# endernewton/tf-faster-rcnn

Measured on AMD Instinct MI355X. Metric: images/sec (600×1000) ResNet-101 Faster R-CNN at 1/2/4/8 MI355X, higher is better.
Workload: dtype f32 (operands, accumulators, results; GEMMs with Cin, Cout % 128 == 0 form each f32 product from two-piece fp16 operands with an exact power-of-two scale per 128-k block on the fp16 matrix pipe -- 3 MFMAs / product, dropped terms <= 3 * 2^-22, measured error vs float64 below the f32-MFMA kernel's; o

## Files before the change

include/frcnn_hip.h:

```cpp
#ifndef FRCNN_HIP_H_
#define FRCNN_HIP_H_
#include <stddef.h>
#include <stdint.h>

#ifdef __cplusplus
extern "C" {
#endif

#define FRCNN_OK 0
#define FRCNN_E_ARG (-1)
#define FRCNN_E_WS (-2)
#define FRCNN_E_UNSUPPORTED (-3)
#define FRCNN_E_HIP(e) (-(1000 + (int)(e)))

#define FRCNN_NMS_RULE_CPU 0
#define FRCNN_NMS_RULE_GPU 1

#define FRCNN_ACT_NONE 0
#define FRCNN_ACT_RELU 1
#define FRCNN_ACT_RELU6 2

#define FRCNN_ABI_VERSION 6
int frcnn_abi_version(void);
const char* frcnn_build_info(void);
// ... 87 lines not shown
int frcnn_box_vote_host(const float* kept , int m, const float* cands , int n, double vote_thresh, float* out );
int frcnn_mirror_views(const float* in_d, int B, int OH, int OW, int c, float* out_d, void* stream);
int frcnn_merge_flip_views(const float* cls_prob_d, const float* bbox_pred_d, const float* rois_d, const int* num_rois_d, int B, int R,
                           int C, float im_w_scaled, float* out_prob_d, float* out_pred_d, float* out_rois_d, int* out_num_d,
                           void* stream);
int frcnn_merge_flip_views_host(const float* cls_prob, const float* bbox_pred, const float* rois, const int* num_rois, int B, int R, int C,
                                float im_w_scaled, float* out_prob, float* out_pred, float* out_rois, int* out_num);

int frcnn_im_detect_boxes(const float* rois_d, const float* bbox_pred_d, int R, int C, double im_scale,
                          int im_h, int im_w, float* boxes_d, void* stream);

int frcnn_bbox_transform_inv(const float* boxes_d, const float* deltas_d, int N, int k, float* out_d, void* stream);
int frcnn_clip_boxes(float* boxes_d, int N, int k, float im_h, float im_w, void* stream);
int frcnn_bbox_transform(const float* ex_rois_d, const float* gt_rois_d, int N, float* targets_d, void* stream);

int frcnn_bbox_overlaps(const double* boxes_d, int n, const double* query_d, int k, double* out_d, void* stream);

size_t frcnn_coco_match_workspace_bytes(int n_groups, long long n_det, long long n_gt, long long n_pairs);
int frcnn_coco_match(const double* det_xywh_d, const long long* det_off_d, const double* gt_xywh_d, const double* gt_area_d,
                     const unsigned char* gt_crowd_d, const long long* gt_off_d, int n_groups, const double* iou_thrs_d, int T,
                     const double* area_rng_d, int A, unsigned char* det_matched_d, unsigned char* det_ignored_d,
                     unsigned char* gt_ignored_d, double* iou_out_d, void* ws, size_t ws_bytes, void* stream);

size_t frcnn_proposal_recall_workspace_bytes(int n_images, long long max_boxes, long long n_gt_total);
int frcnn_proposal_recall(const float* boxes_d, int box_stride, long long n_rows, const long long* start_d, const int* count_d,
                          const float* scale_d, int n_images, long long max_boxes, int limit, const double* gt_d,
                          const long long* gt_off_d, long long n_gt_total, double* gt_iou_d, int* ran_out_d, void* ws, size_t ws_bytes,
                          void* stream);
int frcnn_proposal_recall_host(const float* boxes, int box_stride, long long n_rows, const long long* start, const int* count,
                               const float* scale, int n_images, long long max_boxes, int limit, const double* gt,
                               const long long* gt_off, long long n_gt_total, double* gt_iou, int* ran_out, void* ws, size_t ws_bytes);

int frcnn_conv2d_nhwc(const float* x_d, int N, int H, int W, int Cin, const float* w_d, const float* bias_d,
                      const float* residual_d, int RH, int RW, int res_stride, float* y_d, int OH, int OW,
                      int Cout, int KH, int KW, int stride, int pad_top, int pad_left, int act, int fold_w,
                      void* stream);
size_t frcnn_conv2d_workspace_bytes(int N, int OH, int OW, int Cout, int KH, int KW, int Cin, int fold_w);
int frcnn_conv2d_nhwc_ws(const float* x_d, int N, int H, int W, int Cin, const float* w_d, const float* bias_d,
                         const float* residual_d, int RH, int RW, int res_stride, float* y_d, int OH, int OW, int Cout, int KH,
                         int KW, int stride, int pad_top, int pad_left, int act, int fold_w, void* ws, size_t ws_bytes,
                         void* stream);

int frcnn_set_tuning(int key, int value);
unsigned int frcnn_crc32c(const void* data, size_t n, unsigned int crc);

long long frcnn_snappy_uncompress(const unsigned char* src, size_t n, unsigned char* dst, size_t cap);

int frcnn_prep_image_shape(int h, int w, int target_size, int max_size, double* im_scale, int* out_h, int* out_w);
int frcnn_prep_image(const void* src_d, int src_is_float, int h, int w, const double* pixel_means, double im_scale, float* out_d,
                     int OH, int OW, int out_c, void* stream);
int frcnn_prep_image_batched(const void* src_d, int src_is_float, int B, int h, int w, const double* pixel_means, double im_scale,
                             float* out_d, int OH, int OW, int out_c, void* stream);
int frcnn_prep_train_image(const void* src_d, int src_is_float, int h, int w, int flipped, const double* pixel_means, double im_scale,
                           float* out_d, int OH, int OW, int out_c, const unsigned short* boxes_d, const int* classes_d, int G,
                           float* gt_d, void* stream);

int frcnn_jpeg_info(const unsigned char* data, size_t n, int* out8);
size_t frcnn_jpeg_coef_bytes(int width, int height, int ncomp, int hs, int vs);
int frcnn_jpeg_entropy_decode(const unsigned char* data, size_t n, void* coef_h, size_t coef_bytes);
int frcnn_jpeg_pixels_host(const void* coef_h, int width, int height, int ncomp, int hs, int vs, unsigned char* bgr_h);
size_t frcnn_jpeg_workspace_bytes(int width, int height, int ncomp, int hs, int vs);
int frcnn_jpeg_pixels(const void* coef_d, int width, int height, int ncomp, int hs, int vs, unsigned char* bgr_d, void* ws,
                      size_t ws_bytes, void* stream);

int frcnn_jpeg_quant_tables(int quality, unsigned short* out128);
int frcnn_jpeg_coefs(const unsigned char* bgr_d, int width, int height, int hs, int vs, int quality, void* coef_d, void* ws,
                     size_t ws_bytes, void* stream);
int frcnn_jpeg_coefs_host(const unsigned char* bgr_h, int width, int height, int hs, int vs, int quality, void* coef_h);
size_t frcnn_jpeg_stream_bound(int width, int height, int hs, int vs);
long long frcnn_jpeg_entropy_encode(const void* coef_h, int width, int height, int hs, int vs, unsigned char* out, size_t cap);

int frcnn_draw_detections(unsigned char* bgr_d, int h, int w, const float* dets_d, const int* cnt_d, int max_dets, float conf,
                          int thickness, int scale, const unsigned char* colours_d, int num_colours, const unsigned char* labels_d,
                          int num_classes, int label_stride, const unsigned char* glyphs_d, void* stream);
int frcnn_draw_detections_host(unsigned char* bgr_h, int h, int w, const float* dets_h, int count, int max_dets, float conf,
                               int thickness, int scale, const unsigned char* colours_h, int num_colours, const unsigned char* labels_h,
                               int num_classes, int label_stride, const unsigned char* glyphs_h);

int frcnn_gemm_batched_nt(const float* x_d, const float* w_d, float* y_d, int G, int M, int N, int K, void* stream);
size_t frcnn_gemm_x3_pack_bytes(int G, int N, int K);
int frcnn_gemm_x3_pack(const float* w_d, int G, int N, int K, void* planes_d, void* stream);
int frcnn_gemm_x3(const float* x_d, const void* planes_d, const float* bias_d, const float* res_d, float* y_d, int G, int M, int N,
                  int K, int act, int cfg, int terms, void* stream);
size_t frcnn_h2_planes_bytes(long long rows, int K);
int frcnn_h2_pack_w(const float* w_d, int G, int N, int K, void* planes_d, float* w_inv_d, void* stream);
int frcnn_h2_split(const float* x_d, long long M, int K, void* planes_d, float* inv_d, void* stream);
int frcnn_gemm_h2(const void* x_planes_d, const float* x_inv_d, const void* w_planes_d, const float* w_inv_d, const float* bias_d,
                  const float* res_d, const void* res_planes_d, const float* res_inv_d, float* y_d, void* y_planes_d, float* y_inv_d,
                  int G, int M, int N, int K, int act, int cfg, void* stream);
size_t frcnn_gemm_h2_mean_workspace_bytes(int G, int M, int N);
int frcnn_gemm_h2_mean(const void* x_planes_d, const float* x_inv_d, const void* w_planes_d, const float* w_inv_d, const float* bias_d,
                       const float* res_d, const void* res_planes_d, const float* res_inv_d, int G, int M, int N, int K, int act, int rows,
                       float* mean_out_d, void* ws, size_t ws_bytes, int cfg, void* stream);
int frcnn_winograd_filter_transform(const float* w_hwio, int Cin, int Cout, const float* scale, int m, float* u_out);
int frcnn_winograd_filter_transform_device(const float* w_packed_d, int Cout, int Cin, int m, int transpose_flip, float* u_d,
                                           void* stream);
int frcnn_winograd_input_transform(const float* x_d, int N, int H, int W, int C, int m, float* v_d, void* stream);
int frcnn_winograd_output_transform(const float* m_d, int N, int H, int W, int C, int m, const float* bias_d, int act, float* y_d,
                                    void* stream);
int frcnn_winograd2_conv_x3(const float* x_d, int N, int H, int W, const void* u_planes_d, const float* bias_d, int act, float* y_d,
                            void* stream);
int frcnn_winograd7_filter_transform(const float* w_hwio, int Cin, int Cout, const float* scale, float* u_out);
int frcnn_winograd7_filter_transform_device(const float* w_packed_d, int Cout, int Cin, int transpose_flip, float* u_d, void* stream);
int frcnn_winograd7_input_transform(const float* x_d, int R, int C, float* v_d, void* stream);
int frcnn_winograd7_output_transform(const float* m_d, int R, int C, const float* bias_d, int act, float* y_d, void* stream);
int frcnn_winograd_input_transform_h2(const float* x_d, int N, int H, int W, int C, int m, void* v_planes_d, float* v_inv_d, void* stream);
int frcnn_winograd_output_transform_h2(const float* m_d, int N, int H, int W, int C, int m, const float* bias_d, int act, float* y_d,
                                       void* y_planes_d, float* y_inv_d, void* stream);
int frcnn_winograd7_input_transform_h2(const float* x_d, int R, int C, void* v_planes_d, float* v_inv_d, void* stream);
int frcnn_winograd7_output_transform_h2(const float* m_d, int R, int C, const float* bias_d, int act, float* y_d, void* y_planes_d,
                                        float* y_inv_d, void* stream);
int frcnn_pack_filter_hwio(const float* w_hwio, int KH, int KW, int Cin, int Cout, const float* scale, float* out);
int frcnn_maxpool_nhwc(const float* x_d, int N, int H, int W, int C, int k, int stride, int pad_top,
                       int pad_left, float* y_d, int OH, int OW, void* stream);
int frcnn_dwconv3x3_nhwc(const float* x_d, int N, int H, int W, int C, const float* w_d, const float* bias_d,
                         float* y_d, int OH, int OW, int stride, int pad_top, int pad_left, int act, void* stream);
int frcnn_dwconv3x3_nhwc_h2(const float* x_d, int N, int H, int W, int C, const float* w_d, const float* bias_d, float* y_d,
                            void* y_planes_d, float* y_inv_d, int OH, int OW, int stride, int pad_top, int pad_left, int act, void* stream);
int frcnn_spatial_mean(const float* x_d, int N, int HW, int C, float* y_d, void* stream);
int frcnn_softmax_rows(const float* x_d, int R, int C, int ld, float* y_d, void* stream);
int frcnn_rpn_softmax(const float* score_d, int HW, int A, int ld, float* prob_d, void* stream);
int frcnn_copy_cols(const float* src_d, int R, int ld_src, int col0, int cols, float* dst_d, int ld_dst, void* stream);

size_t frcnn_anchor_target_workspace_bytes(int H, int W, int A, int max_gt);
int frcnn_anchor_target_layer(const float* gt_boxes_d, int G, float im_h, float im_w, int H, int W, int A,
                              int feat_stride, const double* base_d, int rpn_batchsize, double fg_fraction,
                              double pos_overlap, double neg_overlap, long long seed, const double* opts, float* labels_d,
                              float* bbox_targets_d, float* inside_w_d, float* outside_w_d, void* ws,
                              size_t ws_bytes, void* stream);
int frcnn_anchor_target_layer_inject(const float* gt_boxes_d, int G, float im_h, float im_w, int H, int W, int A, int feat_stride,
                                     const double* base_d, int rpn_batchsize, double fg_fraction, double pos_overlap,
                                     double neg_overlap, const int* disable_d, int n_disable, const double* opts, float* labels_d,
                                     float* bbox_targets_d, float* inside_w_d, float* outside_w_d, void* ws, size_t ws_bytes,
                                     void* stream);
int frcnn_proposal_target_layer(const float* rpn_rois_d, const float* rpn_scores_d, int N, const float* gt_boxes_d,
                                int G, int num_classes, int batch_size, double fg_fraction, double fg_thresh,
                                double bg_thresh_hi, double bg_thresh_lo, const double* means4, const double* stds4,
                                long long seed, const double* opts, float* rois_d, float* roi_scores_d, float* labels_d,
                                float* bbox_targets_d, float* inside_w_d, float* outside_w_d, int* counts_d,
                                void* stream);
int frcnn_proposal_target_layer_dn(const float* rpn_rois_d, const float* rpn_scores_d, int max_rois, const int* num_rois_d,
                                   const float* gt_boxes_d, int G, int num_classes, int batch_size, double fg_fraction,
                                   double fg_thresh, double bg_thresh_hi, double bg_thresh_lo, const double* means4,
                                   const double* stds4, long long seed, const double* opts, float* rois_d, float* roi_scores_d,
                                   float* labels_d, float* bbox_targets_d, float* inside_w_d, float* outside_w_d, int* counts_d,
                                   void* stream);
int frcnn_proposal_target_layer_inject(const float* rpn_rois_d, const float* rpn_scores_d, int N, const float* gt_boxes_d, int G,
                                       int num_classes, int batch_size, const int* keep_inds_d, int n_fg, const double* means4,
                                       const double* stds4, const double* opts, float* rois_d, float* roi_scores_d, float* labels_d,
                                       float* bbox_targets_d, float* inside_w_d, float* outside_w_d, void* stream);
size_t frcnn_loss_workspace_bytes(long long elements);
int frcnn_softmax_ce_loss(const float* logits_d, const float* labels_d, int R, int C, int rpn_A, int rpn_H, int rpn_W,
                          float* loss_d, float* dlogits_d, void* ws, size_t ws_bytes, void* stream);
int frcnn_smooth_l1_loss(const float* pred_d, const float* targets_d, const float* inside_w_d, const float* outside_w_d,
                         long long n, float sigma, float mean_divisor, float* loss_d, float* dpred_d, void* ws,
                         size_t ws_bytes, void* stream);

int frcnn_transpose_pad(const float* in_d, int M, int C, float* out_d, int Mp, void* stream);
int frcnn_im2col_t(const float* x_d, int N, int H, int W, int Cin, int OH, int OW, int KH, int KW, int stride,
                   int pad_top, int pad_left, float* out_d, int Mp, void* stream);
int frcnn_flip_transpose_filter(const float* w_d, int Cout, int KH, int KW, int Cin, float* out_d, void* stream);
int frcnn_conv2d_dgrad_strided(const float* dy_d, int N, int OH, int OW, int Cout, const float* w_d, int KH, int KW,
                               int Cin, int stride, int pad_top, int pad_left, float* dx_d, int H, int W,
                               int accumulate, void* stream);
int frcnn_conv2d_wgrad_supported(int Cin, int Cout);
size_t frcnn_conv2d_wgrad_workspace_bytes(int N, int OH, int OW, int Cin, int Cout, int KH, int KW);
int frcnn_conv2d_wgrad(const float* dy_d, const float* x_d, int N, int H, int W, int Cin, int OH, int OW, int Cout, int KH, int KW,
                       int stride, int pad_top, int pad_left, float* dw_d, void* ws, size_t ws_bytes, void* stream);
void frcnn_conv2d_wgrad_set_plan(int tile, int min_workgroups);
size_t frcnn_conv2d_wgrad_h2_workspace_bytes(int N, int OH, int OW, int Cin, int Cout, int KH, int KW);
int frcnn_conv2d_wgrad_h2(const float* dy_d, const float* x_d, int N, int H, int W, int Cin, int OH, int OW, int Cout, int KH, int KW,
                          int stride, int pad_top, int pad_left, float* dw_d, void* ws, size_t ws_bytes, void* stream);
// ... 63 lines not shown
```

tf-faster-rcnn_amd/csrc/gemm_h2.hip:

```cpp
#include "h2_common.h"
#include <mutex>
#include <type_traits>

typedef float f32x16 __attribute__((ext_vector_type(16)));
typedef _Float16 h8 __attribute__((ext_vector_type(8)));

#define LDS_AS __attribute__((address_space(3)))

struct GemmH2Params {
  const unsigned short* x; const float* x_inv; const unsigned short* w; const float* w_inv;
  const float* bias; const float* res; const unsigned short* resp; const float* resp_inv; float* y; unsigned short* yp; float* y_inv;
  int M, N, K, batch, act, nsteps, mtiles, ntiles;
  long long Mtot;
  int wshare;
  const float* mask;
  float* mean_part; int mean_rows;
};

__device__ __forceinline__ void h2_glds16(unsigned voff, const void* sbase, unsigned lds_base) {
  unsigned keep;
  asm volatile(
      "s_mov_b32 %0, m0\n\t"
      "s_mov_b32 m0, %3\n\t"
      "s_nop 0\n\t"
      "global_load_lds_dwordx4 %1, %2\n\t"
      "s_mov_b32 m0, %0"
      : "=&s"(keep)
      : "v"(voff), "s"(sbase), "s"(lds_base)
      : "memory");
}

__device__ __forceinline__ void h2_glds4(unsigned voff, const void* sbase, unsigned lds_base) {
  unsigned keep;
  asm volatile(
      "s_mov_b32 %0, m0\n\t"
      "s_mov_b32 m0, %3\n\t"
      "s_nop 0\n\t"
      "global_load_lds_dword %1, %2\n\t"
      "s_mov_b32 m0, %0"
      : "=&s"(keep)
      : "v"(voff), "s"(sbase), "s"(lds_base)
      : "memory");
}

__device__ __forceinline__ void h2_glds16c(unsigned voff, const void* sbase, unsigned lds_base) {
  asm volatile(
      "s_mov_b32 m0, %2\n\t"
      "s_nop 0\n\t"
      "global_load_lds_dwordx4 %0, %1"
      :
      : "v"(voff), "s"(sbase), "s"(lds_base)
      : "memory");
}
__device__ __forceinline__ void h2_glds4c(unsigned voff, const void* sbase, unsigned lds_base) {
  asm volatile(
      "s_mov_b32 m0, %2\n\t"
      "s_nop 0\n\t"
      "global_load_lds_dword %0, %1"
      :
      : "v"(voff), "s"(sbase), "s"(lds_base)
      : "memory");
}

template <int N>
__device__ __forceinline__ void h2_wait_vmcnt() {
  asm volatile("s_waitcnt vmcnt(%0)" ::"n"(N) : "memory");
}

enum H2Tune : int {
  H2_SCALES_ONCE = 2,
  H2_PINGPONG = 32,
  H2_MASKED = 128,
  H2_LIGHT_BOUNDARY = 256,
  H2_STORE16 = 512,
  H2_DEFERRED = 1024,
#ifdef FRCNN_ABLATION
  H2_NO_MFMA = 2048,
  H2_NO_FRAG = 4096,
  H2_NO_LOAD = 8192,
#endif
};

template <int BM, int BN, int WM, int WN, int NS, int TUNE>
struct H2Lds {
  static constexpr int NW = (BM / WM) * (BN / WN);
  static constexpr bool PP = (TUNE & H2_PINGPONG) != 0;
  static constexpr int XP = BM * 64, WP = BN * 64;
  static constexpr int S_OFF = 2 * XP + 2 * WP;
  static constexpr int STAGE = S_OFF + (PP ? 0 : 1024);
  static constexpr int RED_OFF = NS * STAGE;
  static constexpr int S2_OFF = RED_OFF + (BN / WN) * BM * 4;
  static constexpr int CB_OFF = S2_OFF + (PP ? NW * 512 : (TUNE & H2_SCALES_ONCE) ? 2048 : 0);
  static constexpr int TOTAL = CB_OFF + ((TUNE & H2_LIGHT_BOUNDARY) ? 2 * 2 * BN * 4 : 0);
  static constexpr int RI_OFF = S_OFF + 512;
};

template <int BM, int BN, int WM, int WN, int NS, int WPE = 2, int TUNE = 0>
__global__ __launch_bounds__((BM / WM) * (BN / WN) * 64) __attribute__((amdgpu_waves_per_eu(WPE))) void k_gemm_h2(const GemmH2Params p) {
  constexpr int NW = (BM / WM) * (BN / WN);
  constexpr int TM = WM / 32, TN = WN / 32;
  constexpr int LA = 2 * BM / 16 / NW;
  constexpr int LB = 2 * BN / 16 / NW;
  constexpr int G = LA + LB;
  constexpr int SL = BM / 64;
  constexpr bool ONCE = (TUNE & H2_SCALES_ONCE) != 0;
  constexpr bool PP = (TUNE & H2_PINGPONG) != 0;
  constexpr bool MASKED = (TUNE & H2_MASKED) != 0;
  constexpr bool LTB = (TUNE & H2_LIGHT_BOUNDARY) != 0;
  constexpr bool W21 = (TUNE & H2_STORE16) != 0;
  constexpr bool DE = (TUNE & H2_DEFERRED) != 0;
  using L = H2Lds<BM, BN, WM, WN, NS, TUNE>;
  constexpr int XP = L::XP, WP = L::WP, S_OFF = L::S_OFF, STAGE = L::STAGE, RED_OFF = L::RED_OFF, S2_OFF = L::S2_OFF, CB_OFF = L::CB_OFF, RI_OFF = L::RI_OFF;
  static_assert(!LTB || (!PP && NS == 2 && NW >= 4 && BN % 64 == 0 && BM <= 128), "light boundary: the two-slot one-barrier-per-slab schedule");
  static_assert(!DE || (LTB && W21 && BN == H2_KB), "deferred epilogue: built on the light boundary's LDS constants and counted waits");
  static_assert(!PP || (NW == 8 && NS == 3 && ONCE && BM == 256 && WM == 64 && BN == 128 && WN == 64),
                "ping-pong geometry: 8 waves as 4 (M) x 2 (N), waves 0-3 = the upper half of the rows");
  static_assert((2 * BM / 16) % NW == 0 && (2 * BN / 16) % NW == 0, "tile/wave mismatch");
  static_assert(BM <= 256 && NS >= 2 && NS <= 4, "stage layout");
  static_assert((NS - 2) * (G + SL) <= 63, "vmcnt range");
  extern __shared__ __attribute__((aligned(16))) char smem[];

  const int tid = threadIdx.x, lane = tid & 63;
  const int wave = __builtin_amdgcn_readfirstlane(tid >> 6);
  const int per = p.mtiles * p.ntiles, T = per * p.batch;
  const int xcd = blockIdx.x & 7, wx = blockIdx.x >> 3, W8 = gridDim.x >> 3;
  const int tq = T / 8, tr = T % 8, tn = tq + (xcd < tr ? 1 : 0);
  const int t_end = (xcd < tr ? xcd * (tq + 1) : tr * (tq + 1) + (xcd - tr) * tq) + tn;
  const int tile0 = t_end - tn + wx;
  if (tile0 >= t_end) return;
  const int my_tiles = (t_end - tile0 + W8 - 1) / W8;
  int left = __builtin_amdgcn_readfirstlane(my_tiles * p.nsteps);

  const int wmi = wave / (BN / WN), wni = wave % (BN / WN);
  const int wm0 = wmi * WM, wn0 = wni * WN;
  const int frow = lane & 31, khalf = lane >> 5;

  const size_t xplane = (size_t)p.Mtot * p.K * 2, wplane = (size_t)p.N * p.K * 2;
  unsigned a_off[LA], b_off[LB], s_off[SL];
  const char* i_xb = nullptr; const char* i_wb = nullptr; const char* i_sb = nullptr;
  int i_tile = tile0, i_step = 0, i_par = 0, c_par = 0;
  int i_g = 0, i_bm0 = 0, i_bn0 = 0, i_cpar = 0, c_cpar = 0;
  int pend = 0;
#pragma unroll
  for (int t = 0; t < LB; ++t) {
    const int u = wave * LB + t, plane = u / (BN / 16), row = (u % (BN / 16)) * 16 + (lane >> 2), pos = lane & 3;
    b_off[t] = (unsigned)((size_t)plane * wplane + (size_t)row * p.K * 2 + ((pos ^ ((row >> 2) & 3)) * 16));
  }
  auto tile_coords = [&](int tl, int& g, int& mt, int& nt) {
    g = tl / per;
    const int rem = tl - g * per;
    mt = rem / p.ntiles;
    nt = rem - mt * p.ntiles;
  };
  auto set_tile = [&](int tl) {
    int g, mt, nt;
    tile_coords(tl, g, mt, nt);
    const int bm0 = mt * BM, bn0 = nt * BN;
    const size_t row0 = (size_t)g * p.M + bm0;
    i_g = g; i_bm0 = bm0; i_bn0 = bn0;
    i_xb = (const char*)p.x + row0 * p.K * 2;
    i_wb = (const char*)p.w + ((size_t)(p.wshare ? 0 : g) * 2 * p.N + bn0) * p.K * 2;
    i_sb = (const char*)(p.x_inv + row0);
#pragma unroll
    for (int t = 0; t < LA; ++t) {
      const int u = wave * LA + t, plane = u / (BM / 16), row = (u % (BM / 16)) * 16 + (lane >> 2), pos = lane & 3;
      const int rr = min(row, p.M - 1 - bm0);
      a_off[t] = (unsigned)((size_t)plane * xplane + (size_t)rr * p.K * 2 + ((pos ^ ((row >> 2) & 3)) * 16));
    }
    const long long last = p.Mtot - 1 - (long long)row0;
#pragma unroll
    for (int j = 0; j < SL; ++j) s_off[j] = (unsigned)(min((long long)((PP ? wm0 : j * 64) + lane), last) * 4);
  };
  const unsigned lds0 = (unsigned)(size_t)(LDS_AS char*)smem;
  auto uniform_ptr = [](const char* q) {
    const unsigned long long v = (unsigned long long)q;
    const unsigned lo = __builtin_amdgcn_readfirstlane((unsigned)v), hi = __builtin_amdgcn_readfirstlane((unsigned)(v >> 32));
    return (const char*)(((unsigned long long)hi << 32) | lo);
  };
  auto issue_one = [&](int buf, int t) {
    const unsigned sb = lds0 + (unsigned)(buf * STAGE);
    if constexpr (PP) {
      if (t < LA) h2_glds16c(a_off[t], uniform_ptr(i_xb), __builtin_amdgcn_readfirstlane(sb + (wave * LA + t) * 1024));
      else if (t < G) h2_glds16c(b_off[t - LA], uniform_ptr(i_wb), __builtin_amdgcn_readfirstlane(sb + 2 * XP + (wave * LB + (t - LA)) * 1024));
      else if (t == G && (i_step & 3) == 0) {
        h2_glds4c(s_off[0], uniform_ptr(i_sb), __builtin_amdgcn_readfirstlane(lds0 + S2_OFF + (wave * 2 + i_par) * 256));
        i_par ^= 1;
      }
      return;
    }
    if (t < LA) h2_glds16(a_off[t], uniform_ptr(i_xb), __builtin_amdgcn_readfirstlane(sb + (wave * LA + t) * 1024));
    else if (t < G) h2_glds16(b_off[t - LA], uniform_ptr(i_wb), __builtin_amdgcn_readfirstlane(sb + 2 * XP + (wave * LB + (t - LA)) * 1024));
    else if (wave == 0) {
      const int j = t - G;
      if (!ONCE) h2_glds4(s_off[j], uniform_ptr(i_sb), __builtin_amdgcn_readfirstlane(sb + S_OFF + j * 256));
      else if ((i_step & 3) == 0) {
        h2_glds4(s_off[j], uniform_ptr(i_sb), __builtin_amdgcn_readfirstlane(lds0 + S2_OFF + i_par * 1024 + j * 256));
        if (j == SL - 1) i_par ^= 1;
      }
    }
  };
  static_assert(!ONCE || NS == 2 || PP, "scales-once needs the uncounted wait of the two-stage ring");
  auto issue_advance = [&]() {
    --left;
    if (++i_step == p.nsteps) {
      i_step = 0; i_tile += W8;
      if (left > 0) set_tile(i_tile);
    } else {
      i_xb += 64; i_wb += 64;
      if ((i_step & 3) == 0) i_sb += (size_t)p.Mtot * 4;
    }
  };

  auto issue_cb = [&]() {
    const unsigned cb = lds0 + CB_OFF + i_cpar * (2 * BN * 4);
    if (wave == 1) {
#pragma unroll
      for (int j = 0; j < BN / 64; ++j)
        h2_glds4((unsigned)(lane * 4), uniform_ptr((const char*)(p.w_inv + (size_t)(p.wshare ? 0 : i_g) * p.N + i_bn0 + j * 64)),
                 __builtin_amdgcn_readfirstlane(cb + j * 256));
    }
    if (wave == 2 && p.bias) {
#pragma unroll
      for (int j = 0; j < BN / 64; ++j)
        h2_glds4((unsigned)(lane * 4), uniform_ptr((const char*)(p.bias + i_bn0 + j * 64)), __builtin_amdgcn_readfirstlane(cb + BN * 4 + j * 256));
    }
    if (wave == 3 && p.resp) {
      const char* rb = (const char*)(p.resp_inv + (size_t)(i_bn0 / H2_KB) * p.Mtot + (size_t)i_g * p.M + i_bm0);
#pragma unroll
      for (int j = 0; j < SL; ++j)
        h2_glds4((unsigned)(min(j * 64 + lane, p.M - 1 - i_bm0) * 4), uniform_ptr(rb), __builtin_amdgcn_readfirstlane(lds0 + i_cpar * STAGE + RI_OFF + j * 256));
    }
    i_cpar ^= 1;
  };
  auto wait_pending = [&](int n) {
    if constexpr (DE) {
      if (n >= 32) {
        if (n >= 48) { if (n >= 56) h2_wait_vmcnt<56>(); else h2_wait_vmcnt<48>(); }
        else { if (n >= 40) h2_wait_vmcnt<40>(); else h2_wait_vmcnt<32>(); }
      } else {
        if (n >= 16) { if (n >= 24) h2_wait_vmcnt<24>(); else h2_wait_vmcnt<16>(); }
        else { if (n >= 8) h2_wait_vmcnt<8>(); else h2_wait_vmcnt<0>(); }
      }
      return;
    }
    if (n >= 63) h2_wait_vmcnt<63>();
    else if (n >= 48) h2_wait_vmcnt<48>();
    else if (n >= 32) h2_wait_vmcnt<32>();
    else if (n >= 16) h2_wait_vmcnt<16>();
    else h2_wait_vmcnt<0>();
  };

  f32x16 tot[TM][TN], tmp[TM][TN];
  const int sw = (frow >> 2) & 3;
  const int x_row = (wm0 + frow) * 64, w_row = 2 * XP + (wn0 + frow) * 64;

#ifdef FRCNN_ABLATION
  constexpr bool NO_MFMA = (TUNE & H2_NO_MFMA) != 0, NO_FRAG = (TUNE & H2_NO_FRAG) != 0, NO_LOAD = (TUNE & H2_NO_LOAD) != 0;
#else
  constexpr bool NO_MFMA = false, NO_FRAG = false, NO_LOAD = false;
#endif
  h8 kxh[NO_FRAG ? TM : 1], kxl[NO_FRAG ? TM : 1], kwh[NO_FRAG ? TN : 1], kwl[NO_FRAG ? TN : 1];
  (void)kxh; (void)kxl; (void)kwh; (void)kwl;
  auto slab_mfma = [&](int cur, auto first_c) {
    constexpr bool FIRST = decltype(first_c)::value;
    const char* sb = smem + cur * STAGE;
#pragma unroll
    for (int t = 0; t < 2; ++t) {
      h8 xh[TM], xl[TM], wh[TN], wl[TN];
      if constexpr (NO_FRAG) {
        if (FIRST && t == 0) {
#pragma unroll
          for (int j = 0; j < TN; ++j) {
            const char* q = sb + w_row + j * 32 * 64 + ((khalf ^ sw) * 16);
            kwh[j] = __builtin_bit_cast(h8, *(const uint4*)(q));
            kwl[j] = __builtin_bit_cast(h8, *(const uint4*)(q + WP));
          }
#pragma unroll
          for (int i = 0; i < TM; ++i) {
            const char* q = sb + x_row + i * 32 * 64 + ((khalf ^ sw) * 16);
            kxh[i] = __builtin_bit_cast(h8, *(const uint4*)(q));
            kxl[i] = __builtin_bit_cast(h8, *(const uint4*)(q + XP));
          }
        }
#pragma unroll
        for (int j = 0; j < TN; ++j) { wh[j] = kwh[j]; wl[j] = kwl[j]; asm volatile("" : "+v"(wh[j]), "+v"(wl[j])); }
#pragma unroll
        for (int i = 0; i < TM; ++i) { xh[i] = kxh[i]; xl[i] = kxl[i]; asm volatile("" : "+v"(xh[i]), "+v"(xl[i])); }
      } else {
#pragma unroll
      for (int j = 0; j < TN; ++j) {
        const char* q = sb + w_row + j * 32 * 64 + (((2 * t + khalf) ^ sw) * 16);
        wh[j] = __builtin_bit_cast(h8, *(const uint4*)(q));
        wl[j] = __builtin_bit_cast(h8, *(const uint4*)(q + WP));
      }
#pragma unroll
      for (int i = 0; i < TM; ++i) {
        const char* q = sb + x_row + i * 32 * 64 + (((2 * t + khalf) ^ sw) * 16);
// ... 372 lines not shown
        if (live) ep_rowmax_merge(mx);
      }
      if (live) {
#pragma unroll
        for (int i = 0; i < TM; ++i) ep_store_planes(T, i, mx[i]);
      }
      if (BN / WN > 1) {
        asm volatile("s_waitcnt lgkmcnt(0)" ::: "memory");
        __builtin_amdgcn_s_barrier();
      }
    }
    c_cpar ^= 1;
  };

  constexpr int HALF = (TM + 1) / 2;
  bool have_prev = false;
  TileRef P{0, 0, 0, 0};
  float dmx[TM];
  (void)dmx;
  auto de_piece = [&](auto pos_c) {
    constexpr int POS = decltype(pos_c)::value;
    if constexpr (POS == 0) {
      if (have_prev) {
        ep_scale_act(P);
        ep_mask(P);
        if (p.yp) ep_rowmax_write(dmx);
      }
    } else if constexpr (POS == 1 || POS == 2) {
      constexpr int I0 = POS == 1 ? 0 : HALF, I1 = POS == 1 ? HALF : TM;
      if (have_prev) {
        if (POS == 1 && p.yp && BN / WN > 1) ep_rowmax_merge(dmx);
#pragma unroll
        for (int i = I0; i < I1; ++i) {
          ep_store_f32(P, i);
          if (p.yp) ep_store_planes(P, i, dmx[i]);
        }
      }
#pragma unroll
      for (int i = I0; i < I1; ++i) load_res_raw(i);
    }
  };

  auto slab = [&](auto pos_c, bool fold, bool first_block) {
    constexpr int POS = decltype(pos_c)::value;
    const std::integral_constant<bool, POS == 0> first_c{};
    if constexpr (DE) asm volatile("s_waitcnt lgkmcnt(0)" ::: "memory");
    if constexpr (LTB) {
      wait_pending(pend);
    } else if (left >= 1) {
      if (wave == 0) h2_wait_vmcnt<(NS - 2) * (G + SL)>(); else h2_wait_vmcnt<(NS - 2) * G>();
    } else {
      h2_wait_vmcnt<0>();
    }
    __builtin_amdgcn_s_barrier();
    const bool more = left > 0;
    if (more) {
#pragma unroll
      for (int t = 0; t < (NO_LOAD ? 0 : G + SL); ++t) issue_one(nxt, t);
      if constexpr (LTB) {
        if (i_step == 0) issue_cb();
        pend = 0;
      }
    }
    if constexpr (DE) {
      __builtin_amdgcn_sched_barrier(0);
      if (first_block) de_piece(pos_c);
      __builtin_amdgcn_sched_barrier(0);
    }
    float ainv[TM];
    if (fold) {
      const int soff = ONCE ? S2_OFF + c_par * 1024 : cur * STAGE + S_OFF;
#pragma unroll
      for (int i = 0; i < TM; ++i) ainv[i] = *(const float*)(smem + soff + (wm0 + i * 32 + frow) * 4);
      c_par ^= 1;
    }
    slab_mfma(cur, first_c);
    if (more) {
      issue_advance();
      nxt = nxt + 1 == NS ? 0 : nxt + 1;
    }
    if (fold) {
      if (LTB && first_block) {
        const float* cbp = (const float*)(smem + CB_OFF + c_cpar * (2 * BN * 4));
        if (!p.res && p.resp) {
          typedef unsigned u32x2 __attribute__((ext_vector_type(2)));
#pragma unroll
          for (int i = 0; i < TM; ++i) {
            const float rri = *(const float*)(smem + c_cpar * STAGE + RI_OFF + (wm0 + i * 32 + frow) * 4);
#pragma unroll
            for (int j = 0; j < TN; ++j)
#pragma unroll
              for (int pq = 0; pq < 2; ++pq) {
                unsigned w[8];
#pragma unroll
                for (int e = 0; e < 8; ++e) w[e] = __float_as_uint(tot[i][j][8 * pq + e]);
                const auto h0 = __builtin_amdgcn_permlane32_swap(w[0], w[2], false, false), h1 = __builtin_amdgcn_permlane32_swap(w[1], w[3], false, false);
                const auto l0 = __builtin_amdgcn_permlane32_swap(w[4], w[6], false, false), l1 = __builtin_amdgcn_permlane32_swap(w[5], w[7], false, false);
                const h4 ha = __builtin_bit_cast(h4, u32x2{h0[0], h1[0]}), hb = __builtin_bit_cast(h4, u32x2{h0[1], h1[1]});
                const h4 la = __builtin_bit_cast(h4, u32x2{l0[0], l1[0]}), lb = __builtin_bit_cast(h4, u32x2{l0[1], l1[1]});
#pragma unroll
                for (int e = 0; e < 4; ++e) {
                  tot[i][j][8 * pq + e] = ((float)ha[e] + (float)la[e]) * rri;
                  tot[i][j][8 * pq + 4 + e] = ((float)hb[e] + (float)lb[e]) * rri;
                }
              }
          }
        }
#pragma unroll
        for (int j = 0; j < TN; ++j)
#pragma unroll
          for (int q = 0; q < 4; ++q) {
            const float4 wi = *(const float4*)(cbp + wn0 + j * 32 + 4 * khalf + 8 * q);
            const float4 bv = p.bias ? *(const float4*)(cbp + BN + wn0 + j * 32 + 4 * khalf + 8 * q) : make_float4(0.f, 0.f, 0.f, 0.f);
            const float s0 = __uint_as_float(0x7f000000u - __float_as_uint(wi.x)), s1 = __uint_as_float(0x7f000000u - __float_as_uint(wi.y));
            const float s2 = __uint_as_float(0x7f000000u - __float_as_uint(wi.z)), s3 = __uint_as_float(0x7f000000u - __float_as_uint(wi.w));
#pragma unroll
            for (int i = 0; i < TM; ++i) {
              tot[i][j][4 * q + 0] = __builtin_fmaf(tmp[i][j][4 * q + 0], ainv[i], (tot[i][j][4 * q + 0] + bv.x) * s0);
              tot[i][j][4 * q + 1] = __builtin_fmaf(tmp[i][j][4 * q + 1], ainv[i], (tot[i][j][4 * q + 1] + bv.y) * s1);
              tot[i][j][4 * q + 2] = __builtin_fmaf(tmp[i][j][4 * q + 2], ainv[i], (tot[i][j][4 * q + 2] + bv.z) * s2);
              tot[i][j][4 * q + 3] = __builtin_fmaf(tmp[i][j][4 * q + 3], ainv[i], (tot[i][j][4 * q + 3] + bv.w) * s3);
            }
          }
      } else {
#pragma unroll
        for (int i = 0; i < TM; ++i)
#pragma unroll
          for (int j = 0; j < TN; ++j)
#pragma unroll
            for (int r = 0; r < 16; ++r) tot[i][j][r] = __builtin_fmaf(tmp[i][j][r], ainv[i], tot[i][j][r]);
      }
    }
    cur = cur + 1 == NS ? 0 : cur + 1;
  };

  set_tile(i_tile);
  set_ctile(c_tile);
  if constexpr (PP) {
    const int grp = wave >> 2;
    h8 fxh[2][TM], fxl[2][TM], fwh[2][TN], fwl[2][TN];
    auto seg_barrier = [&]() {
      __builtin_amdgcn_sched_barrier(0);
      __builtin_amdgcn_s_barrier();
      __builtin_amdgcn_sched_barrier(0);
    };
    auto fold = [&]() {
      float ainv[TM];
#pragma unroll
      for (int i = 0; i < TM; ++i) ainv[i] = *(const float*)(smem + S2_OFF + (wave * 2 + c_par) * 256 + (i * 32 + frow) * 4);
      c_par ^= 1;
#pragma unroll
      for (int i = 0; i < TM; ++i)
#pragma unroll
        for (int j = 0; j < TN; ++j)
#pragma unroll
          for (int r = 0; r < 16; ++r) tot[i][j][r] = __builtin_fmaf(tmp[i][j][r], ainv[i], tot[i][j][r]);
    };
    auto pp_mem = [&](auto pos_c, bool fold_prev, bool live) -> bool {
      constexpr int POS = decltype(pos_c)::value;
      const char* sb = smem + cur * STAGE;
      if (live) {
#pragma unroll
        for (int t = 0; t < 2; ++t) {
#pragma unroll
          for (int j = 0; j < TN; ++j) {
            const char* q = sb + w_row + j * 32 * 64 + (((2 * t + khalf) ^ sw) * 16);
            fwh[t][j] = __builtin_bit_cast(h8, *(const uint4*)(q));
            fwl[t][j] = __builtin_bit_cast(h8, *(const uint4*)(q + WP));
          }
#pragma unroll
          for (int i = 0; i < TM; ++i) {
            const char* q = sb + x_row + i * 32 * 64 + (((2 * t + khalf) ^ sw) * 16);
            fxh[t][i] = __builtin_bit_cast(h8, *(const uint4*)(q));
            fxl[t][i] = __builtin_bit_cast(h8, *(const uint4*)(q + XP));
          }
        }
      } else {
#pragma unroll
        for (int t = 0; t < 2; ++t) {
#pragma unroll
          for (int j = 0; j < TN; ++j) asm volatile("" : "=v"(fwh[t][j]), "=v"(fwl[t][j]));
#pragma unroll
          for (int i = 0; i < TM; ++i) asm volatile("" : "=v"(fxh[t][i]), "=v"(fxl[t][i]));
        }
      }
      const bool more = left > 0;
      if (more) {
#pragma unroll
        for (int t = 0; t <= G; ++t) issue_one(nxt, t);
        issue_advance();
        nxt = nxt + 1 == NS ? 0 : nxt + 1;
      }
      if (fold_prev) fold();
      if (grp == 1) {
        if (more) h2_wait_vmcnt<(POS == 2 ? G + 1 : G)>(); else h2_wait_vmcnt<0>();
      }
// ... 9 lines not shown
        for (int t = 0; t < 2; ++t) {
#pragma unroll
          for (int i = 0; i < TM; ++i)
#pragma unroll
            for (int j = 0; j < TN; ++j) {
              if (POS == 0 && t == 0) {
                f32x16 z;
#pragma unroll
                for (int r = 0; r < 16; ++r) z[r] = 0.f;
                tmp[i][j] = __builtin_amdgcn_mfma_f32_32x32x16_f16(fwh[t][j], fxh[t][i], z, 0, 0, 0);
              } else {
                tmp[i][j] = __builtin_amdgcn_mfma_f32_32x32x16_f16(fwh[t][j], fxh[t][i], tmp[i][j], 0, 0, 0);
              }
            }
#pragma unroll
          for (int i = 0; i < TM; ++i)
#pragma unroll
            for (int j = 0; j < TN; ++j) tmp[i][j] = __builtin_amdgcn_mfma_f32_32x32x16_f16(fwl[t][j], fxh[t][i], tmp[i][j], 0, 0, 0);
#pragma unroll
          for (int i = 0; i < TM; ++i)
#pragma unroll
            for (int j = 0; j < TN; ++j) tmp[i][j] = __builtin_amdgcn_mfma_f32_32x32x16_f16(fwh[t][j], fxl[t][i], tmp[i][j], 0, 0, 0);
        }
      }
      __builtin_amdgcn_s_setprio(0);
      if (grp == 0) {
        if (issued) h2_wait_vmcnt<(POS == 2 ? G + 1 : G)>(); else h2_wait_vmcnt<0>();
      }
      cur = cur + 1 == NS ? 0 : cur + 1;
      seg_barrier();
    };
    bool two = false;
#pragma unroll
    for (int s2 = 0; s2 < 2; ++s2) {
      if (left > 0) {
#pragma unroll
        for (int t = 0; t <= G; ++t) issue_one(nxt, t);
        issue_advance();
        nxt = nxt + 1 == NS ? 0 : nxt + 1;
        two = s2 == 1;
      }
    }
    if (two) h2_wait_vmcnt<G>(); else h2_wait_vmcnt<0>();
    seg_barrier();
    if (grp == 1) seg_barrier();
    const int nkb = p.nsteps >> 2;
    for (int tl = 0; tl < my_tiles; ++tl) {
      const bool live = __builtin_amdgcn_readfirstlane(c_bm0 + wm0 < p.M ? 1 : 0) != 0;
      if (live) init_tot();
      else {
#pragma unroll
        for (int i = 0; i < TM; ++i)
#pragma unroll
          for (int j = 0; j < TN; ++j) asm volatile("" : "=v"(tot[i][j]));
      }
      for (int kb = 0; kb < nkb; ++kb) {
        bool is;
        is = pp_mem(std::integral_constant<int, 0>{}, live && kb > 0, live); pp_mfma(std::integral_constant<int, 0>{}, is, live);
        is = pp_mem(std::integral_constant<int, 1>{}, false, live);          pp_mfma(std::integral_constant<int, 1>{}, is, live);
        is = pp_mem(std::integral_constant<int, 2>{}, false, live);          pp_mfma(std::integral_constant<int, 2>{}, is, live);
        is = pp_mem(std::integral_constant<int, 3>{}, false, live);          pp_mfma(std::integral_constant<int, 3>{}, is, live);
      }
      if (live) fold(); else c_par ^= nkb & 1;
      epilogue(live);
      c_tile += W8;
      if (tl + 1 < my_tiles) set_ctile(c_tile);
    }
    if (grp == 0) seg_barrier();
    h2_wait_vmcnt<0>();
    return;
  }
#pragma unroll
  for (int s = 0; s < NS - 1; ++s) {
    if (left > 0) {
#pragma unroll
      for (int t = 0; t < G + SL; ++t) issue_one(nxt, t);
      if constexpr (LTB) {
        if (i_step == 0) issue_cb();
        pend = 0;
      }
      issue_advance();
      nxt = nxt + 1 == NS ? 0 : nxt + 1;
    }
  }
  const int nkb = p.nsteps >> 2;
  for (int tl = 0; tl < my_tiles; ++tl) {
    init_tot();
    for (int kb = 0; kb < nkb; ++kb) {
      slab(std::integral_constant<int, 0>{}, false, kb == 0);
      slab(std::integral_constant<int, 1>{}, false, kb == 0);
      slab(std::integral_constant<int, 2>{}, false, kb == 0);
      slab(std::integral_constant<int, 3>{}, true, kb == 0);
    }
    if constexpr (DE) {
      if (tl + 1 < my_tiles) {
        P = TileRef{c_bm0, c_bn0, c_g, c_cpar};
        have_prev = true;
        c_cpar ^= 1;
        c_tile += W8;
        set_ctile(c_tile);
        continue;
      }
    }
    epilogue(true);
    c_tile += W8;
    if (tl + 1 < my_tiles) set_ctile(c_tile);
  }
  h2_wait_vmcnt<0>();
}

__global__ __launch_bounds__(256) void k_h2_split(const float* __restrict__ x, long long M, int K, unsigned short* __restrict__ planes,
                                                  float* __restrict__ inv_out) {
  const int nkb = K / H2_KB;
  const long long pairs = M * nkb;
  const int sub = threadIdx.x >> 5, l = threadIdx.x & 31;
  for (long long pr = (long long)blockIdx.x * 8 + sub; pr < pairs; pr += (long long)gridDim.x * 8) {
    const long long m = pr / nkb;
    const int kb = (int)(pr - m * nkb);
    const size_t e = (size_t)m * K + (size_t)kb * H2_KB + 4 * l;
    const float4 v = *(const float4*)(x + e);
    float mx = fmaxf(fmaxf(fabsf(v.x), fabsf(v.y)), fmaxf(fabsf(v.z), fabsf(v.w)));
#pragma unroll
    for (int o = 16; o >= 1; o >>= 1) mx = fmaxf(mx, __shfl_xor(mx, o, 64));
    float scale, inv;
    h2_block_scale(mx, scale, inv);
    h4 hh, ll;
    h2_split4(v, scale, hh, ll);
    *(h4*)(planes + e) = hh;
    *(h4*)(planes + (size_t)M * K + e) = ll;
    if (l == 0) inv_out[(size_t)kb * M + m] = inv;
  }
}

__global__ __launch_bounds__(256) void k_h2_pack_w(const float* __restrict__ w, int rows, int N, int K, unsigned short* __restrict__ planes,
                                                   float* __restrict__ inv_out) {
  const int row = blockIdx.x * 4 + (threadIdx.x >> 6), l = threadIdx.x & 63;
  if (row >= rows) return;
  const float* src = w + (size_t)row * K;
  float mx = 0.f;
  for (int k = 4 * l; k < K; k += 256) {
    const float4 v = *(const float4*)(src + k);
    mx = fmaxf(mx, fmaxf(fmaxf(fabsf(v.x), fabsf(v.y)), fmaxf(fabsf(v.z), fabsf(v.w))));
  }
#pragma unroll
  for (int o = 32; o >= 1; o >>= 1) mx = fmaxf(mx, __shfl_xor(mx, o, 64));
  float scale, inv;
  h2_block_scale(fmaxf(mx, 0x1p-40f), scale, inv);
  const int g = row / N, n = row - g * N;
  unsigned short* ph = planes + ((size_t)g * 2 * N + n) * K;
  unsigned short* pl = ph + (size_t)N * K;
  for (int k = 4 * l; k < K; k += 256) {
    const float4 v = *(const float4*)(src + k);
    h4 hh, ll;
    _Float16 a, b;
    h2_split1(v.x, scale, a, b); hh[0] = a; ll[0] = b;
    h2_split1(v.y, scale, a, b); hh[1] = a; ll[1] = b;
    h2_split1(v.z, scale, a, b); hh[2] = a; ll[2] = b;
    h2_split1(v.w, scale, a, b); hh[3] = a; ll[3] = b;
    *(h4*)(ph + k) = hh;
    *(h4*)(pl + k) = ll;
  }
  if (l == 0) inv_out[row] = inv;
}

extern "C" size_t frcnn_h2_planes_bytes(long long rows, int K) {
  if (rows <= 0 || K <= 0) return 0;
// ... 106 lines not shown
    return FRCNN_E_ARG;
  const long long Mtot = (long long)G * M;
  if (K % H2_KB || N % 128 || 4ll * Mtot * K >= (1ll << 32) || 4ll * N * K >= (1ll << 32) || (long long)M * N >= (1ll << 29)) return FRCNN_E_UNSUPPORTED;
  GemmH2Params p = h2_params(x_planes_d, x_inv_d, w_planes_d, w_inv_d, bias_d, res_d, nullptr, nullptr, y_d, y_planes_d, y_inv_d, G, M, N, K, act);
  p.mask = mask_d;
  return run_h2(p, cfg, (hipStream_t)stream);
}

static int run_h2(GemmH2Params& p, int cfg, hipStream_t st) {
  const int G = p.batch, M = p.M, N = p.N, K = p.K;
  if (cfg < 0) {
    const bool classes = cfg == -1;
    if (cfg == -9) cfg = -1;
    const long long mt256 = (M + 255) / 256, t256 = mt256 * (N / 128) * G;
#ifndef FRCNN_H2_PP_MIN_K
#define FRCNN_H2_PP_MIN_K 1024
#endif
    const int pp_min_k = ((cfg == -4 || cfg == -5 || cfg == -6) && !p.mean_part) ? 512 : FRCNN_H2_PP_MIN_K;
    int pp_cfg = (cfg == -3 || cfg == -4 || (cfg == -6 && K < FRCNN_H2_PP_MIN_K)) ? 34 : 21;
    const bool waste256_ok = mt256 * 256 * 100 <= (long long)M * 104;
    bool pp = K >= pp_min_k && waste256_ok && t256 >= 256;
    bool to31 = false;
    if (classes && !p.mean_part && !p.mask) {
      const long long m64 = (M + 63) / 64 * 64;
      const bool waste64_ok = m64 * 100 <= (long long)M * 104;
      const bool products = (FRCNN_H2_PP_CLASSES & 1) && G > 1 && p.y && !p.yp && !p.res && !p.resp && K >= 512 && waste64_ok && t256 >= 256;
      const bool conv3_f32res = (FRCNN_H2_PP_CLASSES & 2) && p.res && p.yp && K == 512 && waste64_ok && t256 >= 256;
      if (conv3_f32res && !pp) pp_cfg = 34;
      pp = pp || products || conv3_f32res;
      to31 = (FRCNN_H2_PP_CLASSES & 4) && p.resp && p.yp && !p.y && K == 512;
    }
    const bool tiny = (long long)((M + 127) / 128) * (N / 128) * G < 150;
    const bool de = cfg != -2 && cfg != -7 && !p.mean_part && !p.mask && ((p.resp && p.yp && !p.y) || cfg == -8) && !to31;
    cfg = pp ? pp_cfg : tiny ? (cfg == -2 ? 12 : (de && cfg == -8) ? 41 : 33) : (cfg == -2 ? 9 : de ? 40 : 31);
  }
  if (p.mean_part && (cfg == 40 || cfg == 41)) cfg = cfg == 40 ? 31 : 33;
  return p.mask ? h2_dispatch<H2_MASKED>(p, cfg, st) : h2_dispatch<0>(p, cfg, st);
}

__global__ __launch_bounds__(256) void k_h2_mean_finish(const float* __restrict__ part, int G, int M, int N4, int rows, float4* __restrict__ out) {
  const long long t = (long long)blockIdx.x * blockDim.x + threadIdx.x;
  const int per = M / rows;
  if (t >= (long long)G * per * N4) return;
  const int n4 = (int)(t % N4);
  const long long gr = t / N4;
  const int g = (int)(gr / per), r = (int)(gr % per);
  const int nblk = (M + 31) >> 5;
  const int row0 = r * rows, row1 = row0 + rows - 1;
  float4 s = make_float4(0.f, 0.f, 0.f, 0.f);
  for (int b = row0 >> 5; b <= (row1 >> 5); ++b) {
    const int which = ((b << 5) / rows == r) ? 0 : 1;
    const float4 v = *(const float4*)(part + (((size_t)g * nblk + b) * 2 + which) * (size_t)N4 * 4 + (size_t)n4 * 4);
    s.x += v.x; s.y += v.y; s.z += v.z; s.w += v.w;
  }
  const float inv = 1.0f / (float)rows;
  out[t] = make_float4(s.x * inv, s.y * inv, s.z * inv, s.w * inv);
}

extern "C" size_t frcnn_gemm_h2_mean_workspace_bytes(int G, int M, int N) {
  if (G <= 0 || M <= 0 || N <= 0) return 256;
  return (size_t)G * (size_t)((M + 31) / 32) * 2 * (size_t)N * sizeof(float);
}

extern "C" int frcnn_gemm_h2_mean(const void* x_planes_d, const float* x_inv_d, const void* w_planes_d, const float* w_inv_d, const float* bias_d,
                                  const float* res_d, const void* res_planes_d, const float* res_inv_d, int G, int M, int N, int K, int act, int rows,
                                  float* mean_out_d, void* ws, size_t ws_bytes, int cfg, void* stream) {
  if (!x_planes_d || !x_inv_d || !w_planes_d || !w_inv_d || !mean_out_d || !ws || G <= 0 || M <= 0 || N <= 0 || K <= 0 || act < 0 || act > 2 ||
      rows <= 0 || (res_d && res_planes_d) || (res_planes_d && !res_inv_d))
    return FRCNN_E_ARG;
  const long long Mtot = (long long)G * M;
  if (K % H2_KB || N % 128 || M % rows || rows < 32 || 4ll * Mtot * K >= (1ll << 32) || 4ll * N * K >= (1ll << 32) || (long long)M * N >= (1ll << 29))
    return FRCNN_E_UNSUPPORTED;
  if (frcnn_gemm_h2_mean_workspace_bytes(G, M, N) > ws_bytes) return FRCNN_E_WS;
  GemmH2Params p = h2_params(x_planes_d, x_inv_d, w_planes_d, w_inv_d, bias_d, res_d, res_planes_d, res_inv_d, nullptr, nullptr, nullptr, G, M, N, K, act);
  p.mean_part = (float*)ws; p.mean_rows = rows; p.wshare = 1;
  hipStream_t st = (hipStream_t)stream;
  const int rc = run_h2(p, cfg, st);
  if (rc) return rc;
  const long long tot = (long long)G * (M / rows) * (N / 4);
  hipLaunchKernelGGL(k_h2_mean_finish, dim3((unsigned)((tot + 255) / 256)), dim3(256), 0, st, (const float*)ws, G, M, N / 4, rows, (float4*)mean_out_d);
  LAUNCH_CHECK();
  return FRCNN_OK;
}
```

tf-faster-rcnn_amd/csrc/gemm_x3.hip:

```cpp
#include "common.h"
#include "x3_mma.h"
#include <mutex>

struct GemmX3Params {
  const float* x; const unsigned short* wp; const float* bias; const float* res; float* y;
  int M, N, K, nsteps, mtiles, ntiles, batch, act;
  long long gx, gwp, gy;
};

template <int BM, int BN, int WM, int WN, int TERMS = 6>
__global__ __launch_bounds__((BM / WM) * (BN / WN) * 64) __attribute__((amdgpu_waves_per_eu(2))) void k_gemm_x3(const GemmX3Params p) {
  constexpr int NW = (BM / WM) * (BN / WN);
  constexpr int TM = WM / 32, TN = WN / 32;
  constexpr int LA = BM / 8 / NW;
  constexpr int LB = 3 * BN / 16 / NW;
  constexpr int G = LA + LB;
  constexpr int A_BYTES = BM * 128, P_BYTES = BN * 64, STAGE = A_BYTES + 3 * P_BYTES;
  static_assert((BM / 8) % NW == 0 && (3 * BN / 16) % NW == 0, "tile/wave mismatch");
  extern __shared__ __attribute__((aligned(16))) char smem[];

  const int tid = threadIdx.x, lane = tid & 63;
  const int wave = __builtin_amdgcn_readfirstlane(tid >> 6);
  const int per = p.mtiles * p.ntiles, T = per * p.batch;
  const int xcd = blockIdx.x & 7, wx = blockIdx.x >> 3, W8 = gridDim.x >> 3;
  const int tq = T / 8, tr = T % 8, tn = tq + (xcd < tr ? 1 : 0);
  const int t_end = (xcd < tr ? xcd * (tq + 1) : tr * (tq + 1) + (xcd - tr) * tq) + tn;
  int tile = __builtin_amdgcn_readfirstlane(t_end - tn + wx);
  if (tile >= t_end) return;

  const int wm0 = (wave / (BN / WN)) * WM, wn0 = (wave % (BN / WN)) * WN;
  int a_lane[LA], b_lane[LB];
#pragma unroll
  for (int t = 0; t < LB; ++t) {
    const int u = wave * LB + t;
    const int plane = u / (BN / 16), row = (u % (BN / 16)) * 16 + (lane >> 2), pos = lane & 3;
    b_lane[t] = ((plane * p.N + row) * p.K) * 2 + ((pos ^ ((row >> 2) & 3)) * 16);
  }
  const float* ia = p.x; const char* ib = (const char*)p.wp;
  int i_bm0 = 0, i_bn0 = 0, i_g = 0;
  auto set_tile = [&](int tl) {
    const int g = tl / per, rem = tl - g * per;
    const int mt = rem / p.ntiles, nt = rem - mt * p.ntiles;
    i_bm0 = mt * BM; i_bn0 = nt * BN; i_g = g;
    ia = p.x + (size_t)g * p.gx + (size_t)i_bm0 * p.K;
    ib = (const char*)(p.wp + (size_t)g * p.gwp + (size_t)i_bn0 * p.K);
#pragma unroll
    for (int t = 0; t < LA; ++t) {
      const int row = (wave * LA + t) * 8 + (lane >> 3);
      a_lane[t] = (min(row, p.M - 1 - i_bm0) * p.K + ((lane & 7) ^ ((row >> 1) & 7)) * 4) * 4;
    }
  };
  const unsigned lds0 = (unsigned)(size_t)(LDS_AS char*)smem;
  auto issue_one = [&](int buf, int t) {
    const unsigned sb = lds0 + (unsigned)(buf * STAGE);
    if (t < LA) glds16((const char*)ia + a_lane[t], __builtin_amdgcn_readfirstlane(sb + (wave * LA + t) * 1024));
    else glds16(ib + b_lane[t - LA], __builtin_amdgcn_readfirstlane(sb + A_BYTES + (wave * LB + (t - LA)) * 1024));
  };
  auto advance_k = [&]() { ia += 32; ib += 64; };
  auto issue_slab = [&](int buf) {
#pragma unroll
    for (int t = 0; t < G; ++t) issue_one(buf, t);
    advance_k();
  };

  f32x16 acc[TM][TN], acs[TM][TN];
  auto zero_acc = [&]() {
#pragma unroll
    for (int i = 0; i < TM; ++i)
#pragma unroll
      for (int j = 0; j < TN; ++j)
#pragma unroll
        for (int r = 0; r < 16; ++r) { acc[i][j][r] = 0.f; acs[i][j][r] = 0.f; }
  };
  zero_acc();
  const int frow = lane & 31, khalf = lane >> 5;
  const int a_sw = (frow >> 1) & 7, b_sw = (frow >> 2) & 3;
  const int a_row = (wm0 + frow) * 128, b_row = A_BYTES + (wn0 + frow) * 64;

  int c_bm0, c_bn0, c_g;
  const int lane_off = (4 * khalf * p.N + frow) * 4;
  auto sub_base = [&](int i, int j) { return (long long)(c_bm0 + wm0 + i * 32) * p.N + (long long)(c_bn0 + wn0 + j * 32); };
  auto row_soff = [&](int r) { return ((r & 3) + 8 * (r >> 2)) * p.N * 4; };
  auto rsrc_of = [&](const float* tensor, long long sbase) {
    const long long left = ((long long)p.M * p.N - sbase) * 4;
    return __builtin_amdgcn_make_buffer_rsrc((void*)(tensor + sbase), 0, (int)max(0ll, min(left, 0x7fffffffll)), 0x00020000);
  };

  auto slab_body = [&](int cur) {
    const int nbuf = cur ^ 1;
    const char* sb = smem + cur * STAGE;
#pragma unroll
    for (int t = 0; t < 2; ++t) {
      bf16x8 ah[TM], am[TM], al[TM], bh[TN], bm[TN], bl[TN];
#pragma unroll
      for (int j = 0; j < TN; ++j) {
        const char* q = sb + b_row + j * 32 * 64 + (((2 * t + khalf) ^ b_sw) * 16);
        bh[j] = __builtin_bit_cast(bf16x8, *(const uint4*)(q));
        bm[j] = __builtin_bit_cast(bf16x8, *(const uint4*)(q + P_BYTES));
        bl[j] = __builtin_bit_cast(bf16x8, *(const uint4*)(q + 2 * P_BYTES));
      }
#pragma unroll
      for (int i = 0; i < TM; ++i) {
        const char* q = sb + a_row + i * 32 * 128;
        const float4 f0 = *(const float4*)(q + (((4 * t + 2 * khalf) ^ a_sw) * 16));
        const float4 f1 = *(const float4*)(q + (((4 * t + 2 * khalf + 1) ^ a_sw) * 16));
        x3_split8(f0, f1, ah[i], am[i], al[i]);
      }
#pragma unroll
      for (int u = (t * G) / 2; u < ((t + 1) * G) / 2; ++u) issue_one(nbuf, u);
#pragma unroll
      for (int i = 0; i < TM; ++i)
#pragma unroll
        for (int j = 0; j < TN; ++j)
          x3_mma16<TERMS>(ah[i], am[i], al[i], bh[j], bm[j], bl[j], acc[i][j], acs[i][j]);
    }
    advance_k();
  };

  const float act_lo = p.act == FRCNN_ACT_NONE ? -__builtin_inff() : 0.f;
  const float act_hi = p.act == FRCNN_ACT_RELU6 ? 6.f : __builtin_inff();
  auto finish = [&](auto res_c) {
    constexpr bool RES = decltype(res_c)::value;
    float* const py = p.y + (size_t)c_g * p.gy;
    int lo = lane_off;
    asm volatile("" : "+v"(lo));
#pragma unroll
    for (int i = 0; i < TM; ++i)
#pragma unroll
      for (int j = 0; j < TN; ++j) {
        const float bv = p.bias ? p.bias[c_bn0 + wn0 + j * 32 + frow] : 0.f;
        const long long sbase = sub_base(i, j);
        float v[16];
        if (RES) {
          const auto rr = rsrc_of(p.res + (size_t)c_g * p.gy, sbase);
#pragma unroll
          for (int r = 0; r < 16; ++r) v[r] = __builtin_bit_cast(float, __builtin_amdgcn_raw_buffer_load_b32(rr, lo + row_soff(r), 0, 0));
        }
#pragma unroll
        for (int r = 0; r < 16; ++r) {
          float t = (acc[i][j][r] + acs[i][j][r]) + bv;
          if (RES) t += v[r];
          v[r] = act_clamp(t, act_lo, act_hi);
        }
        const auto ry = rsrc_of(py, sbase);
#pragma unroll
        for (int r = 0; r < 16; ++r) __builtin_amdgcn_raw_buffer_store_b32(__builtin_bit_cast(unsigned, v[r]), ry, lo + row_soff(r), 0, 0);
      }
  };

  set_tile(tile);
  c_bm0 = i_bm0; c_bn0 = i_bn0; c_g = i_g;
  issue_slab(0);
  int cur = 0, step = 0;
  for (;;) {
    wait_vmcnt<0>();
    __builtin_amdgcn_s_barrier();
    const bool last = step + 1 == p.nsteps;
    int next = tile;
    if (last) {
      next = __builtin_amdgcn_readfirstlane(tile + W8);
      set_tile(next < t_end ? next : tile);
    }
    slab_body(cur);
    cur ^= 1;
    if (!last) { ++step; continue; }
    if (p.res) finish(std::true_type{}); else finish(std::false_type{});
    if (next >= t_end) break;
    zero_acc();
    step = 0; tile = next; c_bm0 = i_bm0; c_bn0 = i_bn0; c_g = i_g;
  }
  wait_vmcnt<0>();
}

__global__ void k_x3_pack(const float* __restrict__ w, long long nk, int G, unsigned short* __restrict__ out) {
  const long long i = (long long)blockIdx.x * blockDim.x + threadIdx.x;
  if (i >= nk * G) return;
  const long long g = i / nk, e = i - g * nk;
  const float x = w[i];
  const __bf16 h = (__bf16)x;
  const float r = x - (float)h;
  const __bf16 m = (__bf16)r;
  const __bf16 l = (__bf16)(r - (float)m);
  unsigned short* o = out + (size_t)g * 3 * nk + e;
  o[0] = __builtin_bit_cast(unsigned short, h); o[nk] = __builtin_bit_cast(unsigned short, m); o[2 * nk] = __builtin_bit_cast(unsigned short, l);
}

extern "C" size_t frcnn_gemm_x3_pack_bytes(int G, int N, int K) {
  if (G <= 0 || N <= 0 || K <= 0) return 0;
  return (size_t)G * 3 * (size_t)N * (size_t)K * sizeof(unsigned short);
}

extern "C" int frcnn_gemm_x3_pack(const float* w_d, int G, int N, int K, void* planes_d, void* stream) {
  if (!w_d || !planes_d || G <= 0 || N <= 0 || K <= 0) return FRCNN_E_ARG;
  const long long nk = (long long)N * K, tot = nk * G;
  hipLaunchKernelGGL(k_x3_pack, dim3((unsigned)((tot + 255) / 256)), dim3(256), 0, (hipStream_t)stream, w_d, nk, G, (unsigned short*)planes_d);
  LAUNCH_CHECK();
  return FRCNN_OK;
}

template <int BM, int BN, int WM, int WN, int TERMS = 6>
static int launch_x3(const GemmX3Params& q, hipStream_t st) {
  constexpr int NT = (BM / WM) * (BN / WN) * 64;
  constexpr size_t lds = 2 * (size_t)(BM * 128 + 3 * BN * 64);
  auto kern = k_gemm_x3<BM, BN, WM, WN, TERMS>;
  static KernelOnce once;
  int slots = 0;
  HIP_TRY(kernel_once(once, (const void*)kern, NT, lds, &slots));
  if (slots < 8 || q.N % BN) return FRCNN_E_UNSUPPORTED;
  GemmX3Params p = q;
  p.mtiles = cdiv(p.M, BM); p.ntiles = p.N / BN; p.nsteps = p.K / 32;
  const long long T = (long long)p.mtiles * p.ntiles * p.batch;
  if (T >= (1ll << 30)) return FRCNN_E_UNSUPPORTED;
  const int grid = (int)min((long long)(slots / 8) * 8, ((T + 7) / 8) * 8);
  hipLaunchKernelGGL(kern, dim3(grid), dim3(NT), lds, st, p);
  LAUNCH_CHECK();
  return FRCNN_OK;
}

extern "C" int frcnn_gemm_x3(const float* x_d, const void* planes_d, const float* bias_d, const float* res_d, float* y_d, int G, int M,
                             int N, int K, int act, int cfg, int terms, void* stream) {
  if (!x_d || !planes_d || !y_d || G <= 0 || M <= 0 || N <= 0 || K <= 0 || act < 0 || act > 2 || (terms != 6 && terms != 9)) return FRCNN_E_ARG;
  if (K % 32 || N % 64 || (long long)M * N >= (1ll << 31) || (long long)N * K >= (1ll << 28) || K >= (1 << 22))
    return FRCNN_E_UNSUPPORTED;
  GemmX3Params p;
  p.x = x_d; p.wp = (const unsigned short*)planes_d; p.bias = bias_d; p.res = res_d; p.y = y_d;
  p.M = M; p.N = N; p.K = K; p.batch = G; p.act = act;
  p.gx = (long long)M * K; p.gwp = 3ll * N * K; p.gy = (long long)M * N;
  p.nsteps = p.mtiles = p.ntiles = 0;
  hipStream_t st = (hipStream_t)stream;
  if (cfg >= 0 && cfg < 10 && (N % 128) && cfg != 6) cfg = -1;
  if (cfg < 0)
    cfg = (N % 128) ? 6 : ((long long)cdiv(M, 128) * (N / 128) * G >= 256) ? 0 : 1;
  if (terms == 9) {
    switch (cfg) {
      case 0: return launch_x3<128, 128, 64, 64, 9>(p, st);
      case 1: return launch_x3<128, 128, 32, 64, 9>(p, st);
      case 6: return launch_x3<128, 64, 64, 32, 9>(p, st);
      default: return FRCNN_E_ARG;
    }
  }
  switch (cfg) {
    case 0: return launch_x3<128, 128, 64, 64>(p, st);
    case 1: return launch_x3<128, 128, 32, 64>(p, st);
    case 2: return launch_x3<64, 128, 32, 64>(p, st);
    case 3: return launch_x3<128, 128, 32, 128>(p, st);
    case 4: return launch_x3<256, 128, 64, 64>(p, st);
    case 5: return launch_x3<128, 256, 64, 64>(p, st);
    case 6: return launch_x3<128, 64, 64, 32>(p, st);
    default: return FRCNN_E_ARG;
  }
}
```

tf-faster-rcnn_amd/frcnn_hip/__init__.py:

```python
import ctypes
import os
from ctypes import c_double, c_float, c_int, c_longlong, c_size_t, c_ulonglong, c_void_p

_PKG = os.path.dirname(os.path.abspath(__file__))
LIB_PATH = os.path.join(_PKG, "libfrcnn_hip.so")
_lib = None

ABI_VERSION = 6
ACT_NONE, ACT_RELU, ACT_RELU6 = 0, 1, 2
NMS_RULE_CPU, NMS_RULE_GPU = 0, 1

_P = c_void_p
SIGNATURES = {
    "frcnn_abi_version": (c_int, []),
    "frcnn_build_info": (ctypes.c_char_p, []),
    "_nms": (None, [_P, _P, _P, c_int, c_int, c_float, c_int]),
    "frcnn_nms_workspace_bytes": (c_size_t, [c_int]),
    "frcnn_nms": (c_int, [_P, c_int, c_double, c_int, _P, _P, _P, c_size_t, _P]),
    "frcnn_nms_sorted": (c_int, [_P, c_int, c_int, c_double, c_int, _P, _P, _P, c_size_t, _P]),
    "frcnn_nms_rule": (c_int, [_P, c_int, c_double, c_int, c_int, _P, _P, _P, c_size_t, _P]),
    "frcnn_nms_sorted_rule": (c_int, [_P, c_int, c_int, c_double, c_int, c_int, _P, _P, _P, c_size_t, _P]),
    "frcnn_generate_anchors": (c_int, [c_int, _P, c_int, _P, c_int, _P]),
    "frcnn_generate_anchors_pre": (c_int, [c_int, c_int, c_int, _P, c_int, _P, _P]),
    "frcnn_proposal_workspace_bytes": (c_size_t, [c_int, c_int, c_int, c_int]),
# ... 46 lines not shown
    "frcnn_conv2d_nhwc": (c_int, [_P, c_int, c_int, c_int, c_int, _P, _P, _P, c_int, c_int, c_int, _P, c_int, c_int,
                                  c_int, c_int, c_int, c_int, c_int, c_int, c_int, c_int, _P]),
    "frcnn_conv2d_workspace_bytes": (c_size_t, [c_int, c_int, c_int, c_int, c_int, c_int, c_int, c_int]),
    "frcnn_conv2d_nhwc_ws": (c_int, [_P, c_int, c_int, c_int, c_int, _P, _P, _P, c_int, c_int, c_int, _P, c_int, c_int,
                                     c_int, c_int, c_int, c_int, c_int, c_int, c_int, c_int, _P, c_size_t, _P]),
    "frcnn_conv2d_nhwc_masked_ws": (c_int, [_P, c_int, c_int, c_int, c_int, _P, _P, _P, c_int, c_int, c_int, _P, c_int, c_int,
                                            c_int, c_int, c_int, c_int, c_int, c_int, c_int, _P, _P, c_size_t, _P]),
    "frcnn_gemm_h2_masked": (c_int, [_P, _P, _P, _P, _P, _P, _P, _P, _P, _P, c_int, c_int, c_int, c_int, c_int, c_int, _P]),
    "frcnn_winograd_output_transform_masked": (c_int, [_P, c_int, c_int, c_int, c_int, c_int, _P, _P, _P, _P, _P]),
    "frcnn_winograd7_output_transform_masked": (c_int, [_P, c_int, c_int, _P, _P, _P, _P, _P]),
    "frcnn_crc32c": (ctypes.c_uint32, [_P, c_size_t, ctypes.c_uint32]),
    "frcnn_snappy_uncompress": (c_longlong, [_P, c_size_t, _P, c_size_t]),
    "frcnn_prep_image_shape": (c_int, [c_int, c_int, c_int, c_int, _P, _P, _P]),
    "frcnn_prep_image": (c_int, [_P, c_int, c_int, c_int, _P, c_double, _P, c_int, c_int, c_int, _P]),
    "frcnn_prep_image_batched": (c_int, [_P, c_int, c_int, c_int, c_int, _P, c_double, _P, c_int, c_int, c_int, _P]),
    "frcnn_prep_train_image": (c_int, [_P, c_int, c_int, c_int, c_int, _P, c_double, _P, c_int, c_int, c_int, _P, _P, c_int, _P, _P]),
    "frcnn_jpeg_info": (c_int, [_P, c_size_t, _P]),
    "frcnn_jpeg_coef_bytes": (c_size_t, [c_int, c_int, c_int, c_int, c_int]),
    "frcnn_jpeg_entropy_decode": (c_int, [_P, c_size_t, _P, c_size_t]),
    "frcnn_jpeg_pixels_host": (c_int, [_P, c_int, c_int, c_int, c_int, c_int, _P]),
    "frcnn_jpeg_workspace_bytes": (c_size_t, [c_int, c_int, c_int, c_int, c_int]),
    "frcnn_jpeg_pixels": (c_int, [_P, c_int, c_int, c_int, c_int, c_int, _P, _P, c_size_t, _P]),
    "frcnn_jpeg_quant_tables": (c_int, [c_int, _P]),
    "frcnn_jpeg_coefs": (c_int, [_P, c_int, c_int, c_int, c_int, c_int, _P, _P, c_size_t, _P]),
    "frcnn_jpeg_coefs_host": (c_int, [_P, c_int, c_int, c_int, c_int, c_int, _P]),
    "frcnn_jpeg_stream_bound": (c_size_t, [c_int, c_int, c_int, c_int]),
    "frcnn_jpeg_entropy_encode": (c_longlong, [_P, c_int, c_int, c_int, c_int, _P, c_size_t]),
    "frcnn_draw_detections": (c_int, [_P, c_int, c_int, _P, _P, c_int, c_float, c_int, c_int, _P, c_int, _P, c_int, c_int, _P, _P]),
    "frcnn_draw_detections_host": (c_int, [_P, c_int, c_int, _P, c_int, c_int, c_float, c_int, c_int, _P, c_int, _P, c_int, c_int, _P]),
    "frcnn_gemm_batched_nt": (c_int,[_P, _P, _P, c_int, c_int, c_int, c_int, _P]),
    "frcnn_winograd_filter_transform": (c_int, [_P, c_int, c_int, _P, c_int, _P]),
    "frcnn_winograd_filter_transform_device": (c_int, [_P, c_int, c_int, c_int, c_int, _P, _P]),
    "frcnn_winograd_input_transform": (c_int, [_P, c_int, c_int, c_int, c_int, c_int, _P, _P]),
    "frcnn_winograd_output_transform": (c_int, [_P, c_int, c_int, c_int, c_int, c_int, _P, c_int, _P, _P]),
    "frcnn_winograd2_conv_x3": (c_int, [_P, c_int, c_int, c_int, _P, _P, c_int, _P, _P]),
    "frcnn_winograd7_filter_transform": (c_int, [_P, c_int, c_int, _P, _P]),
    "frcnn_winograd7_filter_transform_device": (c_int, [_P, c_int, c_int, c_int, _P, _P]),
    "frcnn_winograd7_input_transform": (c_int, [_P, c_int, c_int, _P, _P]),
    "frcnn_winograd7_output_transform": (c_int, [_P, c_int, c_int, _P, c_int, _P, _P]),
    "frcnn_winograd_input_transform_h2": (c_int, [_P, c_int, c_int, c_int, c_int, c_int, _P, _P, _P]),
    "frcnn_winograd_output_transform_h2": (c_int, [_P, c_int, c_int, c_int, c_int, c_int, _P, c_int, _P, _P, _P, _P]),
    "frcnn_winograd7_input_transform_h2": (c_int, [_P, c_int, c_int, _P, _P, _P]),
    "frcnn_winograd7_output_transform_h2": (c_int, [_P, c_int, c_int, _P, c_int, _P, _P, _P, _P]),
    "frcnn_set_tuning": (c_int, [c_int, c_int]),
    "frcnn_pack_filter_hwio": (c_int, [_P, c_int, c_int, c_int, c_int, _P, _P]),
    "frcnn_maxpool_nhwc": (c_int, [_P, c_int, c_int, c_int, c_int, c_int, c_int, c_int, c_int, _P, c_int, c_int, _P]),
    "frcnn_dwconv3x3_nhwc": (c_int, [_P, c_int, c_int, c_int, c_int, _P, _P, _P, c_int, c_int, c_int, c_int, c_int, c_int, _P]),
    "frcnn_dwconv3x3_nhwc_h2": (c_int, [_P, c_int, c_int, c_int, c_int, _P, _P, _P, _P, _P, c_int, c_int, c_int, c_int, c_int, c_int, _P]),
    "frcnn_spatial_mean": (c_int, [_P, c_int, c_int, c_int, _P, _P]),
    "frcnn_softmax_rows": (c_int, [_P, c_int, c_int, c_int, _P, _P]),
    "frcnn_rpn_softmax": (c_int, [_P, c_int, c_int, c_int, _P, _P]),
    "frcnn_copy_cols": (c_int, [_P, c_int, c_int, c_int, c_int, _P, c_int, _P]),
    "frcnn_anchor_target_workspace_bytes": (c_size_t, [c_int, c_int, c_int, c_int]),
    "frcnn_anchor_target_layer": (c_int, [_P, c_int, c_float, c_float, c_int, c_int, c_int, c_int, _P, c_int, c_double, c_double,
                                          c_double, c_longlong, _P, _P, _P, _P, _P, _P, c_size_t, _P]),
    "frcnn_anchor_target_layer_inject": (c_int, [_P, c_int, c_float, c_float, c_int, c_int, c_int, c_int, _P, c_int, c_double, c_double,
                                                 c_double, _P, c_int, _P, _P, _P, _P, _P, _P, c_size_t, _P]),
    "frcnn_proposal_target_layer_inject": (c_int, [_P, _P, c_int, _P, c_int, c_int, c_int, _P, c_int, _P, _P, _P, _P, _P, _P, _P, _P, _P, _P]),
    "frcnn_proposal_target_layer": (c_int, [_P, _P, c_int, _P, c_int, c_int, c_int, c_double, c_double, c_double, c_double, _P, _P,
                                            c_longlong, _P, _P, _P, _P, _P, _P, _P, _P, _P]),
    "frcnn_proposal_target_layer_dn": (c_int, [_P, _P, c_int, _P, _P, c_int, c_int, c_int, c_double, c_double, c_double, c_double, _P, _P,
                                               c_longlong, _P, _P, _P, _P, _P, _P, _P, _P, _P]),
    "frcnn_loss_workspace_bytes": (c_size_t, [c_longlong]),
    "frcnn_softmax_ce_loss": (c_int, [_P, _P, c_int, c_int, c_int, c_int, c_int, _P, _P, _P, c_size_t, _P]),
    "frcnn_smooth_l1_loss": (c_int, [_P, _P, _P, _P, c_longlong, c_float, c_float, _P, _P, _P, c_size_t, _P]),
    "frcnn_transpose_pad": (c_int, [_P, c_int, c_int, _P, c_int, _P]),
    "frcnn_im2col_t": (c_int, [_P, c_int, c_int, c_int, c_int, c_int, c_int, c_int, c_int, c_int, c_int, c_int, _P, c_int, _P]),
    "frcnn_flip_transpose_filter": (c_int, [_P, c_int, c_int, c_int, c_int, _P, _P]),
    "frcnn_conv2d_dgrad_strided": (c_int, [_P, c_int, c_int, c_int, c_int, _P, c_int, c_int, c_int, c_int, c_int, c_int, _P, c_int,
                                           c_int, c_int, _P]),
    "frcnn_conv2d_wgrad_supported": (c_int, [c_int, c_int]),
    "frcnn_conv2d_wgrad_workspace_bytes": (c_size_t, [c_int, c_int, c_int, c_int, c_int, c_int, c_int]),
    "frcnn_conv2d_wgrad": (c_int, [_P, _P, c_int, c_int, c_int, c_int, c_int, c_int, c_int, c_int, c_int, c_int, c_int, c_int, _P, _P,
                                   c_size_t, _P]),
    "frcnn_conv2d_wgrad_set_plan": (None, [c_int, c_int]),
    "frcnn_conv2d_wgrad_h2_workspace_bytes": (c_size_t, [c_int, c_int, c_int, c_int, c_int, c_int, c_int]),
    "frcnn_conv2d_wgrad_h2": (c_int, [_P, _P, c_int, c_int, c_int, c_int, c_int, c_int, c_int, c_int, c_int, c_int, c_int, c_int, _P, _P,
                                      c_size_t, _P]),
    "frcnn_conv2d_wgrad_h2_set_plan": (None, [c_int, c_int]),
    "frcnn_relu_bwd": (c_int, [_P, _P, c_longlong, _P]),
    "frcnn_gemm_x3_pack_bytes": (c_size_t, [c_int, c_int, c_int]),
    "frcnn_gemm_x3_pack": (c_int, [_P, c_int, c_int, c_int, _P, _P]),
    "frcnn_gemm_x3": (c_int, [_P, _P, _P, _P, _P, c_int, c_int, c_int, c_int, c_int, c_int, c_int, _P]),
    "frcnn_h2_planes_bytes": (c_size_t, [c_longlong, c_int]),
    "frcnn_h2_pack_w": (c_int, [_P, c_int, c_int, c_int, _P, _P, _P]),
    "frcnn_h2_split": (c_int, [_P, c_longlong, c_int, _P, _P, _P]),
    "frcnn_gemm_h2": (c_int, [_P, _P, _P, _P, _P, _P, _P, _P, _P, _P, _P, c_int, c_int, c_int, c_int, c_int, c_int, _P]),
    "frcnn_gemm_h2_mean_workspace_bytes": (c_size_t, [c_int, c_int, c_int]),
    "frcnn_gemm_h2_mean": (c_int, [_P, _P, _P, _P, _P, _P, _P, _P, c_int, c_int, c_int, c_int, c_int, c_int, _P, _P, c_size_t, c_int, _P]),
    "frcnn_relu6_bwd": (c_int, [_P, _P, c_longlong, _P]),
    "frcnn_maxpool_bwd": (c_int, [_P, c_int, c_int, c_int, c_int, c_int, c_int, _P, _P, c_int, c_int, _P, _P]),
    "frcnn_dropout": (c_int, [_P, c_longlong, c_ulonglong, c_float, _P, _P]),
    "frcnn_dwconv3x3_dgrad": (c_int, [_P, c_int, c_int, c_int, c_int, _P, _P, c_int, c_int, c_int, c_int, c_int, c_int, _P]),
    "frcnn_dwconv3x3_wgrad_workspace_bytes": (c_size_t, [c_int, c_int, c_int, c_int]),
    "frcnn_dwconv3x3_wgrad": (c_int, [_P, _P, c_int, c_int, c_int, c_int, c_int, c_int, c_int, c_int, c_int, _P, _P, _P, c_size_t, _P]),
    "frcnn_dwconv3x3_refold": (c_int, [_P, _P, c_int, _P, _P]),
    "frcnn_add_strided": (c_int, [_P, c_int, c_int, c_int, c_int, _P, c_int, c_int, c_int, c_int, _P]),
    "frcnn_spatial_mean_bwd": (c_int, [_P, c_int, c_int, c_int, _P, _P]),
    "frcnn_colsum": (c_int, [_P, c_int, c_int, _P, _P]),
    "frcnn_crop_and_resize_bwd": (c_int, [_P, c_int, c_int, c_int, _P, c_int, c_float, c_int, _P, _P]),
    "frcnn_crop_and_resize_bwd_plan": (c_int, [_P, c_int, c_int, c_int, _P, c_int, c_float, c_int, _P, c_size_t, _P]),
    "frcnn_sgd_momentum": (c_int, [_P, _P, _P, _P, _P, c_longlong, c_int, c_float, c_float, c_float, c_float, _P]),
    "frcnn_sgd_desc_bytes": (c_size_t, []),
    "frcnn_sgd_momentum_multi": (c_int, [_P, c_int, c_float, c_float, c_float, _P]),
    "frcnn_sgd_momentum_range": (c_int, [_P, c_int, c_int, c_float, c_float, c_float, _P]),
    "frcnn_sumsq": (c_int, [_P, c_longlong, c_double, _P, c_int, _P, c_size_t, _P]),
    "frcnn_sumsq_multi": (c_int, [_P, _P, c_int, c_double, _P, c_int, _P, c_size_t, _P]),
    "frcnn_summary_limits": (c_int, [_P]),
    "frcnn_summary_stats_workspace_bytes": (c_size_t, [c_int]),
    "frcnn_summary_stats": (c_int, [_P, c_int, _P, _P, c_size_t, _P]),
    "frcnn_graph_begin": (c_int, [_P]),
    "frcnn_graph_end": (c_int, [_P, ctypes.POINTER(c_void_p)]),
    "frcnn_graph_launch": (c_int, [_P, _P]),
    "frcnn_graph_destroy": (c_int, [_P]),
}


class FrcnnHipError(RuntimeError):
    pass


def lib():
    global _lib
    if _lib is None:
        if not os.path.exists(LIB_PATH):
            raise ImportError("libfrcnn_hip.so not built: run `python -c 'import __graft_entry__ as g; g.build()'` "
                              "(or python tf-faster-rcnn_amd/frcnn_hip/build.py); there is no CPU fallback")
        L = ctypes.CDLL(LIB_PATH)
        for name, (res, args) in SIGNATURES.items():
            fn = getattr(L, name)
            fn.restype, fn.argtypes = res, args
        got = L.frcnn_abi_version()
        if got != ABI_VERSION:
            raise ImportError("libfrcnn_hip.so has ABI version %d, this binding is written for %d: rebuild (python -m frcnn_hip.build)"
                              % (got, ABI_VERSION))
        _lib = L
    return _lib


def check(rc, what):
    if rc != 0:
        if rc <= -1000:
            raise FrcnnHipError("%s: HIP error %d" % (what, -rc - 1000))
        raise FrcnnHipError("%s: %s" % (what, {-1: "bad argument", -2: "workspace too small",
                                               -3: "shape not supported by the kernels"}.get(rc, "error %d" % rc)))


recorder = None


def call(name, *args):
    fn = getattr(lib(), name)
    check(fn(*args), name)
    if recorder is not None:
        recorder.add_call(fn, name, args)
```

tf-faster-rcnn_amd/frcnn_hip/ops.py:

```python
import ctypes

import numpy as np
import torch

import frcnn_hip as _binding
from . import ACT_NONE, NMS_RULE_CPU, call, check, lib

_ws_cache = {}
ws_scope = "default"

_scope_stack = [(None, None, None)]


def active_store(owner, default=None):
    o, _, store = _scope_stack[-1]
    return store if store is not None and (owner is None or o is owner) else default


def scope_depth():
    return len(_scope_stack) - 1


class unscoped(object):

# ... 1057 lines not shown
    dev, n = pred.device, pred.numel()
    loss = _zeros((1,), dtype=torch.float32, device=dev)
    grad = _empty(tuple(pred.shape), dtype=pred.dtype, device=pred.device)
    ws = workspace(lib().frcnn_loss_workspace_bytes(n), dev, "loss")
    call("frcnn_smooth_l1_loss", _ptr(pred), _ptr(targets), _ptr(inside_w), _ptr(outside_w), n, float(sigma), float(mean_divisor),
         _ptr(loss), _ptr(grad), _ptr(ws), ws.numel(), _stream())
    return loss, grad


def transpose_pad(x2d, Mp, out=None):
    _chk(x2d)
    M, C = x2d.shape
    out = _empty((C, Mp), dtype=torch.float32, device=x2d.device) if out is None else out
    call("frcnn_transpose_pad", _ptr(x2d), M, C, _ptr(out), int(Mp), _stream())
    return out


def im2col_t(x, KH, KW, stride, pad, OH, OW, Mp, out=None):
    _chk(x)
    N, H, W, Cin = x.shape
    out = _empty((KH * KW * Cin, Mp), dtype=torch.float32, device=x.device) if out is None else out
    call("frcnn_im2col_t", _ptr(x), N, H, W, Cin, OH, OW, KH, KW, int(stride), int(pad[0]), int(pad[2]), _ptr(out), int(Mp), _stream())
    return out


def flip_transpose_filter(w_packed, out=None):
    _chk(w_packed)
    Cout, KH, KW, Cin = w_packed.shape
    out = _empty((Cin, KH, KW, Cout), dtype=torch.float32, device=w_packed.device) if out is None else out
    call("frcnn_flip_transpose_filter", _ptr(w_packed), Cout, KH, KW, Cin, _ptr(out), _stream())
    return out


def conv2d_dgrad_strided(dy, w_packed, stride, pad, H, W, dx, accumulate):
    _chk(dy), _chk(w_packed), _chk(dx)
    N, OH, OW, Cout = dy.shape
    _, KH, KW, Cin = w_packed.shape
    call("frcnn_conv2d_dgrad_strided", _ptr(dy), N, OH, OW, Cout, _ptr(w_packed), KH, KW, Cin, int(stride), int(pad[0]), int(pad[2]),
         _ptr(dx), int(H), int(W), 1 if accumulate else 0, _stream())
    return dx


def conv2d_wgrad_supported(Cin, Cout):
    return bool(lib().frcnn_conv2d_wgrad_supported(int(Cin), int(Cout)))


def conv2d_wgrad(dy, x, KH, KW, stride, pad, out, h2=False):
    _chk(dy), _chk(x), _chk(out)
    N, OH, OW, Cout = dy.shape
    _, H, W, Cin = x.shape
    if out.numel() != Cout * KH * KW * Cin:
        raise ValueError("conv2d_wgrad: out has %d elements, the filter %d" % (out.numel(), Cout * KH * KW * Cin))
    name = "frcnn_conv2d_wgrad_h2" if h2 else "frcnn_conv2d_wgrad"
    nb = getattr(lib(), name + "_workspace_bytes")(N, OH, OW, Cin, Cout, int(KH), int(KW))
    ws = workspace(nb, x.device, "conv_wgrad") if nb else None
    call(name, _ptr(dy), _ptr(x), N, H, W, Cin, OH, OW, Cout, int(KH), int(KW), int(stride), int(pad[0]), int(pad[2]),
         _ptr(out), _ptr(ws), int(nb), _stream())
    return out


def relu_bwd(grad, y):
    _chk(grad), _chk(y)
    call("frcnn_relu_bwd", _ptr(grad), _ptr(y), grad.numel(), _stream())
    return grad


def gemm_x3_pack(w, planes=None):
    _chk(w)
    G, N, K = (w.shape[0], w.shape[1], w.shape[2]) if w.dim() == 3 else (1, w.shape[0], w[0].numel())
    if planes is None:
        planes = torch.empty(lib().frcnn_gemm_x3_pack_bytes(G, N, K), dtype=torch.uint8, device=w.device)
    call("frcnn_gemm_x3_pack", _ptr(w), G, N, K, _ptr(planes), _stream())
    return planes


def gemm_x3(x, planes, G, M, N, K, bias=None, residual=None, act=ACT_NONE, out=None, cfg=-1, terms=6):
    _chk(x)
    out = _empty((G, M, N) if G > 1 else (M, N), dtype=torch.float32, device=x.device) if out is None else out
    call("frcnn_gemm_x3", _ptr(x), _ptr(planes), _ptr(bias), _ptr(residual), _ptr(out), int(G), int(M), int(N), int(K), int(act),
         int(cfg), int(terms), _stream())
    return out


class H2(object):
    __slots__ = ("planes", "inv", "rows", "K")

    def __init__(self, planes, inv, rows, K):
        self.planes, self.inv, self.rows, self.K = planes, inv, int(rows), int(K)

    @staticmethod
    def empty(rows, K, device):
        assert K % 128 == 0
        return H2(torch.empty(lib().frcnn_h2_planes_bytes(int(rows), int(K)), dtype=torch.uint8, device=device),
                  torch.empty((K // 128, rows), dtype=torch.float32, device=device), rows, K)

    def to_float(self):
        hl = self.planes.view(torch.float16).view(2, self.rows, self.K).float()
        inv = self.inv.t().repeat_interleave(128, dim=1)
        return (hl[0] + hl[1]) * inv


def h2_split(x, out=None):
    _chk(x)
    K = x.shape[-1]
    rows = x.numel() // K
    out = H2.empty(rows, K, x.device) if out is None else out
    assert out.rows == rows and out.K == K
    call("frcnn_h2_split", _ptr(x), rows, K, _ptr(out.planes), _ptr(out.inv), _stream())
    return out


def h2_pack_w(w, out=None):
    _chk(w)
    G, N, K = (w.shape[0], w.shape[1], w.shape[2]) if w.dim() == 3 else (1, w.shape[0], w[0].numel())
    if out is None:
        out = (torch.empty(lib().frcnn_h2_planes_bytes(G * N, K), dtype=torch.uint8, device=w.device),
               torch.empty((G, N), dtype=torch.float32, device=w.device))
    call("frcnn_h2_pack_w", _ptr(w), G, N, K, _ptr(out[0]), _ptr(out[1]), _stream())
    return out


def gemm_h2(x, wp, G, M, N, K, bias=None, residual=None, act=ACT_NONE, out=None, out_planes=None, want_f32=True, cfg=-1, mask=None):
    assert isinstance(x, H2) and x.rows == G * M and x.K == K
    if out is None and want_f32:
        out = _empty((G * M, N), dtype=torch.float32, device=x.planes.device)
    if out_planes is not None:
        assert out_planes.rows == G * M and out_planes.K == N
    rp = residual if isinstance(residual, H2) else None
    if rp is not None:
        assert rp.rows == G * M and rp.K == N
    if mask is not None:
        _chk(mask)
        assert rp is None and mask.numel() == G * M * N
        call("frcnn_gemm_h2_masked", _ptr(x.planes), _ptr(x.inv), _ptr(wp[0]), _ptr(wp[1]), _ptr(bias), _ptr(residual), _ptr(mask), _ptr(out),
             _ptr(None if out_planes is None else out_planes.planes), _ptr(None if out_planes is None else out_planes.inv),
             int(G), int(M), int(N), int(K), int(act), int(cfg), _stream())
        return out, out_planes
    call("frcnn_gemm_h2", _ptr(x.planes), _ptr(x.inv), _ptr(wp[0]), _ptr(wp[1]), _ptr(bias), _ptr(None if rp is not None else residual),
         _ptr(None if rp is None else rp.planes), _ptr(None if rp is None else rp.inv), _ptr(out),
         _ptr(None if out_planes is None else out_planes.planes), _ptr(None if out_planes is None else out_planes.inv),
         int(G), int(M), int(N), int(K), int(act), int(cfg), _stream())
    return out, out_planes


def gemm_h2_mean(x, wp, G, M, N, K, bias, residual, act, rows, out=None, cfg=-1):
    assert isinstance(x, H2) and x.rows == G * M and x.K == K and M % rows == 0
    if out is None:
        out = _empty((G * (M // rows), N), dtype=torch.float32, device=x.planes.device)
    rp = residual if isinstance(residual, H2) else None
    ws = workspace(lib().frcnn_gemm_h2_mean_workspace_bytes(int(G), int(M), int(N)), x.planes.device, "h2_mean")
    call("frcnn_gemm_h2_mean", _ptr(x.planes), _ptr(x.inv), _ptr(wp[0]), _ptr(wp[1]), _ptr(bias), _ptr(None if rp is not None else residual),
         _ptr(None if rp is None else rp.planes), _ptr(None if rp is None else rp.inv), int(G), int(M), int(N), int(K), int(act), int(rows),
         _ptr(out), _ptr(ws), ws.numel() * ws.element_size(), int(cfg), _stream())
    return out


def winograd_input_transform_h2(x, v, m):
    _chk(x)
    N, H, W, C = x.shape
    assert isinstance(v, H2) and v.K == C and v.rows == winograd_points(m) * winograd_tiles(N, H, W, m)
    if m == 7:
        call("frcnn_winograd7_input_transform_h2", _ptr(x), N, C, _ptr(v.planes), _ptr(v.inv), _stream())
    else:
        call("frcnn_winograd_input_transform_h2", _ptr(x), N, H, W, C, int(m), _ptr(v.planes), _ptr(v.inv), _stream())
    return v


def winograd_output_transform_h2(mm, bias, act, shape, m, out_planes, out=None):
    _chk(mm)
    N, H, W, C = shape
    assert isinstance(out_planes, H2) and out_planes.rows == N * H * W and out_planes.K == C
    assert mm.numel() == winograd_points(m) * winograd_tiles(N, H, W, m) * C
    if out is not None:
        _chk(out)
        assert tuple(out.shape) == tuple(shape)
    if m == 7:
        call("frcnn_winograd7_output_transform_h2", _ptr(mm), N, C, _ptr(bias), int(act), _ptr(out), _ptr(out_planes.planes),
             _ptr(out_planes.inv), _stream())
    else:
        call("frcnn_winograd_output_transform_h2", _ptr(mm), N, H, W, C, int(m), _ptr(bias), int(act), _ptr(out), _ptr(out_planes.planes),
             _ptr(out_planes.inv), _stream())
    return out_planes


def relu6_bwd(grad, y):
    _chk(grad), _chk(y)
    call("frcnn_relu6_bwd", _ptr(grad), _ptr(y), grad.numel(), _stream())
    return grad


def maxpool_bwd(x, y, dy, k, stride, dx):
    _chk(x), _chk(y), _chk(dy), _chk(dx)
    N, H, W, C = x.shape
    call("frcnn_maxpool_bwd", _ptr(x), N, H, W, C, int(k), int(stride), _ptr(y), _ptr(dy), y.shape[1], y.shape[2], _ptr(dx), _stream())
    return dx


def dropout(x, seed, keep_prob, out=None, step_mult=0):
    _chk(x)
    out = _empty(tuple(x.shape), dtype=x.dtype, device=x.device) if out is None else out
    call("frcnn_dropout", _ptr(x), x.numel(), int(seed) & 0xFFFFFFFFFFFFFFFF, float(keep_prob), _ptr(out), _stream())
    if _binding.recorder is not None and step_mult:
        _binding.recorder.patch_last(2, step_mult)
    return out


def dwconv3x3_dgrad(g, w, stride, pad, dx, accumulate=False):
    _chk(g), _chk(w), _chk(dx)
    N, OH, OW, C = g.shape
    call("frcnn_dwconv3x3_dgrad", _ptr(g), N, OH, OW, C, _ptr(w), _ptr(dx), dx.shape[1], dx.shape[2], int(stride), int(pad[0]), int(pad[2]),
         1 if accumulate else 0, _stream())
    return dx


def dwconv3x3_wgrad(g, x, stride, pad, scale, dw):
    _chk(g), _chk(x), _chk(dw)
    N, OH, OW, C = g.shape
    ws = workspace(lib().frcnn_dwconv3x3_wgrad_workspace_bytes(N, OH, OW, C), g.device, "dw_wgrad")
    call("frcnn_dwconv3x3_wgrad", _ptr(g), _ptr(x), N, x.shape[1], x.shape[2], C, OH, OW, int(stride), int(pad[0]), int(pad[2]), _ptr(scale),
         _ptr(dw), _ptr(ws), ws.numel(), _stream())
    return dw


def dwconv3x3_refold(w, scale, wf):
    _chk(w), _chk(scale), _chk(wf)
    call("frcnn_dwconv3x3_refold", _ptr(w), _ptr(scale), w.shape[-1], _ptr(wf), _stream())
    return wf
# ... 142 lines not shown
```

tf-faster-rcnn_amd/lib/model/config.py:

```python
import ast
import os
import os.path as osp

import numpy as np


class AttrDict(dict):

    def __init__(self, d=None, **kw):
        super().__init__()
        for k, v in dict(d or {}, **kw).items():
            self[k] = v

    def __setitem__(self, k, v):
        if isinstance(v, dict) and not isinstance(v, AttrDict):
            v = AttrDict(v)
        super().__setitem__(k, v)

    def __getattr__(self, k):
        try:
            return self[k]
        except KeyError:
            raise AttributeError(k)

    __setattr__ = __setitem__


_TRAIN = dict(
    LEARNING_RATE=0.001, MOMENTUM=0.9, WEIGHT_DECAY=0.0001, GAMMA=0.1, STEPSIZE=[30000], DISPLAY=10,
    DOUBLE_BIAS=True, TRUNCATED=False, BIAS_DECAY=False, USE_GT=False, ASPECT_GROUPING=False,
    SNAPSHOT_KEPT=3, SUMMARY_INTERVAL=180, SCALES=(600,), MAX_SIZE=1000, IMS_PER_BATCH=1, BATCH_SIZE=128,
    FG_FRACTION=0.25, FG_THRESH=0.5, BG_THRESH_HI=0.5, BG_THRESH_LO=0.1, USE_FLIPPED=True, BBOX_REG=True,
    BBOX_THRESH=0.5, SNAPSHOT_ITERS=5000, SNAPSHOT_PREFIX='res101_faster_rcnn', BBOX_NORMALIZE_TARGETS=True,
    BBOX_INSIDE_WEIGHTS=(1.0, 1.0, 1.0, 1.0), BBOX_NORMALIZE_TARGETS_PRECOMPUTED=True,
    BBOX_NORMALIZE_MEANS=(0.0, 0.0, 0.0, 0.0), BBOX_NORMALIZE_STDS=(0.1, 0.1, 0.2, 0.2), PROPOSAL_METHOD='gt',
    HAS_RPN=True, RPN_POSITIVE_OVERLAP=0.7, RPN_NEGATIVE_OVERLAP=0.3, RPN_CLOBBER_POSITIVES=False,
    RPN_FG_FRACTION=0.5, RPN_BATCHSIZE=256, RPN_NMS_THRESH=0.7, RPN_PRE_NMS_TOP_N=12000,
    RPN_POST_NMS_TOP_N=2000, RPN_BBOX_INSIDE_WEIGHTS=(1.0, 1.0, 1.0, 1.0), RPN_POSITIVE_WEIGHT=-1.0,
    USE_ALL_GT=True)

_TEST = dict(
    SCALES=(600,), MAX_SIZE=1000, NMS=0.3, SVM=False, BBOX_REG=True, HAS_RPN=False, PROPOSAL_METHOD='gt',
    RPN_NMS_THRESH=0.7, RPN_PRE_NMS_TOP_N=6000, RPN_POST_NMS_TOP_N=300, MODE='nms', RPN_TOP_N=5000)

__C = AttrDict(
    TRAIN=_TRAIN, TEST=_TEST,
    RESNET=dict(MAX_POOL=False, FIXED_BLOCKS=1),
    MOBILENET=dict(REGU_DEPTH=False, FIXED_LAYERS=5, WEIGHT_DECAY=0.00004, DEPTH_MULTIPLIER=1.),
    PIXEL_MEANS=np.array([[[102.9801, 115.9465, 122.7717]]]), RNG_SEED=3,
    ROOT_DIR=osp.abspath(osp.join(osp.dirname(__file__), '..', '..')),
    MATLAB='matlab', EXP_DIR='default', USE_GPU_NMS=True, USE_E2E_TF=False, POOLING_MODE='crop', POOLING_SIZE=7,
    ANCHOR_SCALES=[8, 16, 32], ANCHOR_RATIOS=[0.5, 1, 2], RPN_CHANNELS=512,
    HIP=dict(WINOGRAD=True, WINOGRAD_MIN_CIN=64, WINOGRAD_M=4, WINOGRAD_F2_SCOPES=("block1", "block2"), WINOGRAD_DIRECT_SCOPES=(),
             WINOGRAD_TRAIN=True, WINOGRAD_DGRAD=True,
             WINOGRAD_7X7=True, WINOGRAD_FUSED_F2=True, FUSE_TAIL_MEAN=True, MFMA_X3=True,
             MFMA_H2=True, H2_LAZY_SPLIT=True, H2_MIN_TILES=150, H2_TRAIN_MIN_TILES=320, H2_TRUNK_PLANES=True, H2_TILE_CFG=-1,
             X3_TILE_CFG=-1, H2_TRAIN=True, WGRAD_STREAM=2, WGRAD_TN=True, WGRAD_H2=True, PREP_STREAM=True, TRAIN_REPLAY=True, TRAIN_PICK_STREAMS=6,
             GRAPH_CACHE_SHAPES=4, TRAIN_CACHE_SHAPES=16, JPEG_DEVICE=False, TEST_BATCH_IMAGES=1,
             SOFT_NMS=0, SOFT_NMS_SIGMA=0.5, SOFT_NMS_MIN_SCORE=0.001, TEST_FLIP=False, BBOX_VOTE=False, BBOX_VOTE_THRESH=0.8))
__C.DATA_DIR = osp.abspath(osp.join(__C.ROOT_DIR, 'data'))
cfg = __C


def get_output_dir(imdb, weights_filename):
    outdir = osp.abspath(osp.join(__C.ROOT_DIR, 'output', __C.EXP_DIR, imdb.name))
    outdir = osp.join(outdir, 'default' if weights_filename is None else weights_filename)
    os.makedirs(outdir, exist_ok=True)
    return outdir


def get_output_tb_dir(imdb, weights_filename):
    outdir = osp.abspath(osp.join(__C.ROOT_DIR, 'tensorboard', __C.EXP_DIR, imdb.name))
    outdir = osp.join(outdir, 'default' if weights_filename is None else weights_filename)
    os.makedirs(outdir, exist_ok=True)
    return outdir


_NULLABLE_KEYS = ("H2_TRAIN_MIN_TILES",)


def _merge_a_into_b(a, b):
    if not isinstance(a, dict):
        return
    for k, v in a.items():
        if k not in b:
            raise KeyError('{} is not a valid config key'.format(k))
        old = b[k]
        if type(old) is not type(v) and not (isinstance(old, dict) and isinstance(v, dict)):
            if isinstance(old, np.ndarray):
                v = np.array(v, dtype=old.dtype)
            elif isinstance(old, tuple) and isinstance(v, list):
                v = tuple(v)
            elif isinstance(old, list) and isinstance(v, tuple):
                v = list(v)
            elif k in _NULLABLE_KEYS and (v is None or old is None) and isinstance(old if v is None else v, int):
                pass
            else:
                raise ValueError('Type mismatch ({} vs. {}) for config key: {}'.format(type(old), type(v), k))
        if isinstance(v, dict):
            try:
                _merge_a_into_b(v, b[k])
            except Exception:
                print('Error under config key: {}'.format(k))
                raise
        else:
            b[k] = v


def cfg_from_file(filename):
    import yaml
    with open(filename, 'r') as f:
        _merge_a_into_b(AttrDict(yaml.safe_load(f) or {}), __C)


def cfg_from_list(cfg_list):
    assert len(cfg_list) % 2 == 0
    for k, v in zip(cfg_list[0::2], cfg_list[1::2]):
        path = k.split('.')
        d = __C
        for sub in path[:-1]:
            assert sub in d
            d = d[sub]
        leaf = path[-1]
        assert leaf in d
        try:
            value = ast.literal_eval(v)
        except Exception:
            value = v
        old = d[leaf]
        if isinstance(old, tuple) and isinstance(value, list):
            value = tuple(value)
        if isinstance(old, list) and isinstance(value, tuple):
            value = list(value)
        nullable = leaf in _NULLABLE_KEYS and (value is None or old is None) and isinstance(old if value is None else value, int)
        assert nullable or type(value) == type(old), 'type {} does not match original type {}'.format(type(value), type(old))
        d[leaf] = value
```

tf-faster-rcnn_amd/lib/nets/network.py:

```python
import collections

import numpy as np
import torch

from frcnn_hip import ACT_NONE, ACT_RELU, NMS_RULE_CPU, NMS_RULE_GPU, ops
from frcnn_hip.runtime import VarSpec
from model.config import cfg


class Network(object):
    def __init__(self):
        self._predictions = {}
        self._losses = {}
        self._anchor_targets = {}
        self._proposal_targets = {}
        self._layers = {}
        self._act_summaries = []
        self._variables_to_fix = {}
        self._feat_stride = [16, ]
        self._scope = "network"
        self._sess = None
        self._image = None
        self._im_info = None
        self._var_specs = collections.OrderedDict()
# ... 26 lines not shown
    def _declare_backbone(self):
        raise NotImplementedError

    def _head_channels(self):
        raise NotImplementedError

    def _tail_channels(self):
        raise NotImplementedError

    def variable_specs(self):
        return self._var_specs

    def _conv(self, x, scope, k, stride=1, pad=(0, 0, 0, 0), act=ACT_RELU, bn_eps=None, residual=None,
              res_stride=1, fold_w=False, out_affine=None, real_cin=None, no_bias=False, emit_h2=False, want_f32=True):
        sess = self._sess
        N, H, W, Cin = x.shape
        wino = (cfg.HIP.WINOGRAD and k == 3 and stride == 1 and tuple(pad) == (1, 1, 1, 1)
                and residual is None and not fold_w and out_affine is None and not no_bias
                and Cin % 32 == 0 and Cin >= cfg.HIP.WINOGRAD_MIN_CIN and act in (ACT_NONE, ACT_RELU)
                and not any(tok in scope for tok in cfg.HIP.WINOGRAD_DIRECT_SCOPES))
        if wino and self._mode == "TEST":
            return self._conv_winograd(x, scope, act, bn_eps, emit_h2, want_f32)
        wino = wino and cfg.HIP.WINOGRAD_TRAIN
        w, b = sess.conv_params(scope, bn_eps=bn_eps, fold_w=fold_w,
                                out_scale=None if out_affine is None else out_affine[0],
                                out_shift=None if out_affine is None else out_affine[1])
        if no_bias:
            b = None
        N, H, W, Cin = x.shape
        OH = ops.conv_out_size(H, k, stride, pad[0], pad[1])
        OW = ops.conv_out_size(W, k, stride, pad[2], pad[3])
        Cout = w.shape[0]
        out = sess.buf(self._tag + "/" + scope, (N, OH, OW, Cout))
        flops = 2 * N * OH * OW * Cout * k * k * (Cin if real_cin is None else real_cin)
        plain = k == 1 and stride == 1 and tuple(pad) == (0, 0, 0, 0) and not fold_w and (residual is None or res_stride == 1)
        M = N * OH * OW
        if wino:
            m = self._winograd_scheme(scope, H, W)
            G, T = ops.winograd_points(m), ops.winograd_tiles(N, H, W, m)
            u = sess.prepared.get(("fwd", "wino_u", self._tag, scope, m), lambda: ops.winograd_filter_transform_device(
                w, m, False, out=sess.buf(self._tag + "/wino_u/" + scope, (G, Cout, Cin))))
            mm = sess.buf(self._tag + "/wino_m", (G, T, Cout))
            v = sess.buf(self._tag + "/wino_v", (G, T, Cin))
            yp = sess.h2_buf(self._tag + "/" + scope, M, Cout) if (emit_h2 and cfg.HIP.MFMA_H2 and Cout % 128 == 0) else None
            sess.mark("conv:" + scope, 2 * G * T * Cout * Cin,
                      lambda: ops.conv3x3_winograd(x, u, b, act, out=out, v_buf=v, m_buf=mm, out_planes=yp),
                      nbytes=4 * (v.numel() + u.numel() + mm.numel()))
            self._wrote(out, yp, True) if yp is not None else self._wrote(out)
        elif plain and self._h2_eligible(M, Cout, Cin, 1, scope) and self._h2_input(x) is not None:
            xp, wp = self._h2_input(x), sess.h2_planes(w)
            yp = sess.h2_buf(self._tag + "/" + scope, M, Cout) if emit_h2 else None
            y = out if (want_f32 or yp is None or self._mode == "TRAIN") else None
            res = residual
            if residual is not None and residual.data_ptr() in self._f32_missing:
                res = self._h2_of[residual.data_ptr()]
            tcfg = int(cfg.HIP.H2_TILE_CFG)
            sess.mark("conv:h2:" + scope, flops, lambda: ops.gemm_h2(xp, wp, 1, M, Cout, Cin, b, res, act, out=y, out_planes=yp,
                                                                      want_f32=False, cfg=tcfg),
                      nbytes=4 * M * Cin + 4 * w.numel() + (4 * out.numel() if y is not None else 0)
                      + (4 * out.numel() if yp is not None else 0) + (4 * out.numel() if residual is not None else 0))
            self._wrote(out, yp, y is not None)
        elif plain and self._x3_eligible(M, Cout, Cin, 1):
            self._need_f32(x), self._need_f32(residual)
            planes = sess.x3_planes(w)
            xc = int(cfg.HIP.X3_TILE_CFG)
            sess.mark("conv:x3:" + scope, flops, lambda: ops.gemm_x3(x, planes, 1, M, Cout, Cin, b, residual, act, out=out, cfg=xc),
                      nbytes=4 * (x.numel() + out.numel() + (out.numel() if residual is not None else 0)) + 6 * w.numel())
            self._wrote(out)
        else:
            self._need_f32(x), self._need_f32(residual)
            sess.mark("conv:" + scope, flops,
                      lambda: ops.conv2d(x, w, b, k, k, stride, pad, act, residual, res_stride, fold_w, out=out),
                      nbytes=4 * (x.numel() + w.numel() + out.numel() + (out.numel() if residual is not None else 0)))
            self._wrote(out)
        if self._mode == "TRAIN":
            self._tape.append(dict(kind="conv", scope=scope, x=x, y=out, k=k, stride=stride, pad=tuple(pad), act=act,
                                   residual=residual, res_stride=res_stride))
            if self.trainable_scope(scope) or x.data_ptr() in self._requires_grad:
                self._requires_grad.add(out.data_ptr())
            if residual is not None and residual.data_ptr() in self._requires_grad:
                self._requires_grad.add(out.data_ptr())
        return out

    H2_MIN_CHANNEL_RATIO = 2.0 ** -18

    def _h2_eligible(self, M, N, K, G, scope=None):
        rows = G * M
        if scope is not None and self._mode == "TEST" and self._sess.h2_channel_spread(scope) < self.H2_MIN_CHANNEL_RATIO:
            return False
        return (bool(cfg.HIP.MFMA_H2) and (self._mode == "TEST" or bool(cfg.HIP.H2_TRAIN)) and K % 128 == 0 and N % 128 == 0
                and ((self._plan_rows(M) + 127) // 128) * (N // 128) * G >= self._h2_min_tiles()
                and 4 * rows * K < (1 << 32) and 4 * N * K < (1 << 32) and M * N < (1 << 29))

    @staticmethod
    def h2_min_tiles(mode):
        if mode == "TRAIN" and cfg.HIP.H2_TRAIN_MIN_TILES is not None:
            return int(cfg.HIP.H2_TRAIN_MIN_TILES)
        return int(cfg.HIP.H2_MIN_TILES)

    def _h2_min_tiles(self):
        return self.h2_min_tiles(self._mode)

    def _h2_input(self, x):
        xp = self._h2_of.get(x.data_ptr())
        if xp is None and cfg.HIP.H2_LAZY_SPLIT:
            self._need_f32(x)
            K = x.shape[-1]
            xp = self._sess.h2_buf(self._tag + "/split@%x" % x.data_ptr(), x.numel() // K, K)
            self._sess.mark("op:h2_split", 0, lambda: ops.h2_split(x, out=xp), nbytes=8 * x.numel())
            self._h2_of[x.data_ptr()] = xp
        return xp

    def _wrote(self, t, planes=None, f32=True):
        k = t.data_ptr()
        if planes is None:
            self._h2_of.pop(k, None)
        else:
            self._h2_of[k] = planes
        (self._f32_missing.discard if f32 else self._f32_missing.add)(k)
        return t

    def _need_f32(self, x):
        if x is not None and x.data_ptr() in self._f32_missing:
            raise RuntimeError("graph construction error: a float32 consumer reads a tensor that was emitted as operand planes only")

    def _x3_eligible(self, M, N, K, G):
        return (bool(cfg.HIP.MFMA_X3) and self._mode == "TEST" and N % 64 == 0 and K % 32 == 0
                and ((self._plan_rows(M) + 127) // 128) * ((N + 127) // 128) * G >= 150 and M * N < (1 << 31) and N * K < (1 << 28))

    @staticmethod
    def _winograd_scheme(scope, H, W):
        if any(tok in scope for tok in cfg.HIP.WINOGRAD_F2_SCOPES):
            return 2
        m = int(cfg.HIP.WINOGRAD_M)
        return 7 if (m == 4 and H == 7 and W == 7 and cfg.HIP.WINOGRAD_7X7) else m

    def _conv_winograd(self, x, scope, act, bn_eps, emit_h2=False, want_f32=True):
        sess = self._sess
        self._need_f32(x)
        N, H, W, Cin = x.shape
        m = self._winograd_scheme(scope, H, W)
        u, b = sess.winograd_params(scope, bn_eps=bn_eps, m=m)
        G, Cout = u.shape[0], u.shape[1]
        T = ops.winograd_tiles(N, H, W, m)
        out = sess.buf(self._tag + "/" + scope, (N, H, W, Cout))
        flops = 2 * G * T * Cout * Cin
        if (cfg.HIP.WINOGRAD_FUSED_F2 and m == 2 and Cin == 64 and Cout == 64 and self._mode == "TEST" and self._x3_eligible(T, Cout, Cin, G)
                and N * H * W < (1 << 23)):
            planes = sess.x3_planes(u)
            sess.mark("conv:x3:" + scope, flops, lambda: ops.winograd2_conv_x3(x, planes, b, act, out),
                      nbytes=4 * (x.numel() + out.numel()) + 6 * u.numel())
            return self._wrote(out)
        mm = sess.buf(self._tag + "/wino_m", (G, T, Cout))
        if self._h2_eligible(T, Cout, Cin, G, scope):
            vp, wp = sess.h2_buf(self._tag + "/wino_v", G * T, Cin), sess.h2_planes(u)
            sess.mark("op:wino_in", 0, lambda: ops.winograd_input_transform_h2(x, vp, m), nbytes=4 * (x.numel() + G * T * Cin))
            tcfg = int(cfg.HIP.H2_TILE_CFG)
            sess.mark("conv:h2:" + scope, flops, lambda: ops.gemm_h2(vp, wp, G, T, Cout, Cin, out=mm, cfg=tcfg),
                      nbytes=4 * (G * T * Cin + mm.numel()) + 4 * u.numel())
        else:
            v = sess.buf(self._tag + "/wino_v", (G, T, Cin))
            sess.mark("op:wino_in", 0, lambda: ops.winograd_input_transform(x, v, m), nbytes=4 * (x.numel() + v.numel()))
            if self._x3_eligible(T, Cout, Cin, G):
                planes = sess.x3_planes(u)
                xc = int(cfg.HIP.X3_TILE_CFG)
                sess.mark("conv:x3:" + scope, flops, lambda: ops.gemm_x3(v, planes, G, T, Cout, Cin, out=mm, cfg=xc),
# ... 308 lines not shown

    _trainable_on_device = False

    @staticmethod
    def _check_supported_cfg(mode):
        t = cfg.TRAIN
        fixed = [("POOLING_MODE", cfg.POOLING_MODE, "crop")]
        bad = ["%s = %r (only %r is implemented)" % (k, v, want) for k, v, want in fixed if v != want]
        if float(t.RPN_POSITIVE_WEIGHT) >= 0 and not (0.0 < float(t.RPN_POSITIVE_WEIGHT) < 1.0):
            bad.append("TRAIN.RPN_POSITIVE_WEIGHT = %r (the reference asserts 0 < p < 1, anchor_target_layer.py:103-104)" % (t.RPN_POSITIVE_WEIGHT,))
        h = cfg.HIP
        if h.SOFT_NMS not in (0, 1, 2):
            bad.append("HIP.SOFT_NMS = %r (0 = hard NMS, 1 = linear, 2 = Gaussian)" % (h.SOFT_NMS,))
        if not float(h.SOFT_NMS_SIGMA) > 0:
            bad.append("HIP.SOFT_NMS_SIGMA = %r (must be > 0)" % (h.SOFT_NMS_SIGMA,))
        if not float(h.SOFT_NMS_MIN_SCORE) >= 0:
            bad.append("HIP.SOFT_NMS_MIN_SCORE = %r (must be >= 0)" % (h.SOFT_NMS_MIN_SCORE,))
        if not 0.0 < float(h.BBOX_VOTE_THRESH) <= 1.0:
            bad.append("HIP.BBOX_VOTE_THRESH = %r (must be in (0, 1])" % (h.BBOX_VOTE_THRESH,))
        if h.TEST_FLIP and mode == "TEST":
            bad += Network._flip_refusals()
        if bad:
            raise NotImplementedError("unsupported configuration for the HIP path: " + "; ".join(bad))

    FLIP_MAX_ROWS = 1024

    @staticmethod
    def _flip_refusals():
        bad = []
        if cfg.TEST.MODE != "nms":
            bad.append("HIP.TEST_FLIP with TEST.MODE = %r (the flip ensemble merges the 'nms' proposals of two views)" % (cfg.TEST.MODE,))
        elif 2 * int(cfg.TEST.RPN_POST_NMS_TOP_N) > Network.FLIP_MAX_ROWS:
            bad.append("HIP.TEST_FLIP with TEST.RPN_POST_NMS_TOP_N = %d (two views give %d rows per image, the post-processing holds at most %d)"
                       % (int(cfg.TEST.RPN_POST_NMS_TOP_N), 2 * int(cfg.TEST.RPN_POST_NMS_TOP_N), Network.FLIP_MAX_ROWS))
        return bad

    def create_architecture(self, mode, num_classes, tag=None, anchor_scales=(8, 16, 32), anchor_ratios=(0.5, 1, 2)):
        assert tag is not None
        self._check_supported_cfg(mode)
        if mode == "TRAIN" and not self._trainable_on_device:
            raise NotImplementedError("%s: no reverse sweep for this network's TRAIN graph; TEST mode works" % type(self).__name__)
        self._tag = tag
        self._num_classes = num_classes
        self._mode = mode
        self._anchor_scales = tuple(anchor_scales)
        self._num_scales = len(anchor_scales)
        self._anchor_ratios = tuple(anchor_ratios)
        self._num_ratios = len(anchor_ratios)
        self._num_anchors = self._num_scales * self._num_ratios
        A = self._num_anchors
        self._var_specs.clear()
        self._declare_backbone()
        hc = self._head_channels()
        self._declare_conv_bias(self._scope + "/rpn_conv/3x3", 3, 3, hc, cfg.RPN_CHANNELS, 0.01)
        self._declare_conv_bias(self._scope + "/rpn_cls_score", 1, 1, cfg.RPN_CHANNELS, 2 * A, 0.01)
        self._declare_conv_bias(self._scope + "/rpn_bbox_pred", 1, 1, cfg.RPN_CHANNELS, 4 * A, 0.01)
        tc = self._tail_channels()
        self._var(self._scope + "/cls_score/weights", (tc, num_classes), "normal", 0.01)
        self._var(self._scope + "/cls_score/biases", (num_classes,), "zeros")
        self._var(self._scope + "/bbox_pred/weights", (tc, 4 * num_classes), "normal", 0.001)
        self._var(self._scope + "/bbox_pred/biases", (4 * num_classes,), "zeros")
        names = ["rois", "rpn_cls_score", "rpn_cls_prob", "rpn_bbox_pred", "cls_score", "cls_prob", "bbox_pred"]
        return {k: k for k in names}

    def _stage_image(self, sess, image, im_info=None):
        if isinstance(image, np.ndarray):
            image = torch.from_numpy(np.ascontiguousarray(image, dtype=np.float32))
        B, H, W, C = image.shape
        if im_info is None:
            buf = sess.buf(self._tag + "/image", (B, H, W, 4), zero=True)
        else:
            with self.shape_scope(sess, (B, H, W, 4), im_info):
                buf = sess.buf(self._tag + "/image", (B, H, W, 4), zero=True)
        buf[..., :C].copy_(image, non_blocking=True)
        return buf

    def graph_key(self, image_shape, im_info):
        c = cfg[self._mode]
        return (self._tag, self._scope, self._num_classes, self._anchor_scales, self._anchor_ratios, bool(cfg.RESNET.MAX_POOL),
                bool(cfg.USE_GPU_NMS), tuple(int(v) for v in image_shape), (float(im_info[0]), float(im_info[1])), self._mode, cfg.TEST.MODE, self._fuse_tail_entry,
                c.RPN_PRE_NMS_TOP_N, c.RPN_POST_NMS_TOP_N, c.RPN_NMS_THRESH, cfg.TEST.RPN_TOP_N, cfg.POOLING_SIZE,
                bool(cfg.HIP.WINOGRAD), int(cfg.HIP.WINOGRAD_MIN_CIN), int(cfg.HIP.WINOGRAD_M), tuple(cfg.HIP.WINOGRAD_F2_SCOPES),
                tuple(cfg.HIP.WINOGRAD_DIRECT_SCOPES), bool(cfg.HIP.WINOGRAD_7X7), bool(cfg.HIP.FUSE_TAIL_MEAN), bool(cfg.HIP.MFMA_X3), bool(cfg.USE_E2E_TF),
                bool(cfg.HIP.MFMA_H2), bool(cfg.HIP.H2_LAZY_SPLIT), int(cfg.HIP.H2_MIN_TILES), bool(cfg.HIP.H2_TRUNK_PLANES), int(cfg.HIP.H2_TILE_CFG), int(cfg.HIP.X3_TILE_CFG), bool(cfg.HIP.H2_TRAIN))

    def shape_scope(self, sess, image_shape, im_info):
        return sess.shape_scope(self.graph_key(image_shape, im_info), group=("graphs", self._tag), cap=int(cfg.HIP.GRAPH_CACHE_SHAPES))

    def forward_device(self, sess, image_d, im_info, use_graph=True):
        self._sess = sess
        self._image = image_d
        self._im_info = (float(im_info[0]), float(im_info[1]), float(im_info[2]))
        sess.prepared.wait_planes()
        ops.ws_scope = self._tag
        key = self.graph_key(image_d.shape, self._im_info)
        cur = torch.cuda.current_stream(sess.device)
        with self.shape_scope(sess, image_d.shape, self._im_info):
            if not use_graph or sess.profile is not None:
                sess.flops_last_forward = 0
                self._build_network(self._mode == "TRAIN")
                return self._predictions
            if key not in sess.graphs:
                with torch.cuda.stream(sess.stream):
                    sess.stream.wait_stream(cur)
                    sess.flops_last_forward = 0
                    self._build_network(False)
                    sess.stream.synchronize()
                    flops = sess.flops_last_forward
                    g = ops.Graph().capture(lambda: self._build_network(False))
                    sess.stream.synchronize()
                sess.graphs[key] = (g, dict(self._predictions), self._num_rois, flops, self._rois_per_image, image_d)
            g, preds, num, flops, per, captured = sess.graphs[key]
            self._predictions, self._num_rois, sess.flops_last_forward, self._rois_per_image = dict(preds), num, flops, per
            if captured.data_ptr() != image_d.data_ptr():
                captured.copy_(image_d, non_blocking=True)
            g.launch()
        return self._predictions

    def _build_proposals(self):
        with self._plan_context(self, False):
            self._tape = []
            self._requires_grad = set()
            self._act_summaries = []
            self._h2_of, self._f32_missing = {}, set()
            net_conv = self._image_to_head(False)
            self._anchor_component()
            rois = self._region_proposal(net_conv, False)
        B, per, s = int(self._image.shape[0]), self._rois_per_image, self._sess
        if self._num_rois is None:
            return rois, s.buf(self._tag + "/top_scores", (per, 1)), torch.full((B,), per, dtype=torch.int32, device=rois.device)
        return rois, s.buf(self._tag + "/roi_scores", (B * per, 1)), self._num_rois

    def propose_device(self, sess, image_d, im_info, use_graph=True):
        assert self._mode == "TEST", "propose_device is a test-time path"
        self._sess = sess
        self._image = image_d
        self._im_info = (float(im_info[0]), float(im_info[1]), float(im_info[2]))
        sess.prepared.wait_planes()
        ops.ws_scope = self._tag
        scope_key = self.graph_key(image_d.shape, self._im_info)
        key = ("propose",) + scope_key
        cur = torch.cuda.current_stream(sess.device)
        with self.shape_scope(sess, image_d.shape, self._im_info):
            if not use_graph or sess.profile is not None or cfg.TEST.MODE != "nms":
                sess.flops_last_forward = 0
                return self._build_proposals()
            ent = sess.graphs.get(key)
            if ent is None:
                with torch.cuda.stream(sess.stream):
                    sess.stream.wait_stream(cur)
                    sess.flops_last_forward = 0
                    out = self._build_proposals()
                    sess.stream.synchronize()
                    flops = sess.flops_last_forward
                    g = ops.Graph().capture(self._build_proposals)
                    sess.stream.synchronize()
                ent = sess.graphs[key] = dict(scope=scope_key, graph=g, out=out, flops=flops, per=self._rois_per_image, image=image_d)
            self._num_rois, sess.flops_last_forward, self._rois_per_image = ent["out"][2], ent["flops"], ent["per"]
            if ent["image"].data_ptr() != image_d.data_ptr():
                ent["image"].copy_(image_d, non_blocking=True)
            ent["graph"].launch()
        return ent["out"]

    def extract_head(self, sess, image):
        self._sess = sess
        sess.prepared.wait_planes()
        shape = (int(image.shape[0]), int(image.shape[1]), int(image.shape[2]), 4)
# ... 346 lines not shown
```

tf-faster-rcnn_amd/lib/nets/resnet_v1.py:

```python
from frcnn_hip import ACT_NONE, ACT_RELU, ops
from model.config import cfg
from nets.network import Network

BN_EPS = 1e-5


def _same_pad(k, stride):
    total = k - 1
    beg = total // 2
    return (beg, total - beg, beg, total - beg)


class resnetv1(Network):
    _rgb_first_conv = "/conv1"
    _trainable_on_device = True
    def __init__(self, num_layers=50):
        Network.__init__(self)
        self._feat_stride = [16, ]
        self._feat_compress = [1. / float(self._feat_stride[0]), ]
        self._num_layers = num_layers
        self._scope = 'resnet_v1_%d' % num_layers
        self._decide_blocks()

    def _decide_blocks(self):
        units = {50: (3, 4, 6, 3), 101: (3, 4, 23, 3), 152: (3, 8, 36, 3)}.get(self._num_layers)
        if units is None:
            raise NotImplementedError
        self._blocks = [("block1", 64, units[0], 2), ("block2", 128, units[1], 2),
                        ("block3", 256, units[2], 1),
                        ("block4", 512, units[3], 1)]

    def _declare_backbone(self):
        s = self._scope
        self._declare_conv_bn(s + "/conv1", 7, 7, 3, 64)
        cin = 64
        for name, base, n_units, _ in self._blocks:
            depth = base * 4
            for u in range(1, n_units + 1):
                p = "%s/%s/unit_%d/bottleneck_v1" % (s, name, u)
                if cin != depth:
                    self._declare_conv_bn(p + "/shortcut", 1, 1, cin, depth)
                self._declare_conv_bn(p + "/conv1", 1, 1, cin, base)
                self._declare_conv_bn(p + "/conv2", 3, 3, base, base)
                self._declare_conv_bn(p + "/conv3", 1, 1, base, depth, residual_branch_end=True)
                cin = depth

    def _head_channels(self):
        return self._blocks[2][1] * 4

    def _tail_channels(self):
        return self._blocks[3][1] * 4

    def _bottleneck(self, x, prefix, base, stride, mean_rows=0, emit_out=True, f32_out=True):
        depth = base * 4
        cin = x.shape[-1]
        if cin != depth:
            shortcut = self._conv(x, prefix + "/shortcut", 1, stride, act=ACT_NONE, bn_eps=BN_EPS)
            res_stride = 1
        else:
            shortcut, res_stride = x, stride
        r = self._conv(x, prefix + "/conv1", 1, 1, act=ACT_RELU, bn_eps=BN_EPS)
        pad = (1, 1, 1, 1) if stride == 1 else _same_pad(3, stride)
        N, H, W, _ = r.shape
        M3 = N * ops.conv_out_size(H, 3, stride, pad[0], pad[1]) * ops.conv_out_size(W, 3, stride, pad[2], pad[3])
        if mean_rows and res_stride == 1 and stride == 1 and self._mean_fusable(M3, depth, base, prefix + "/conv3", mean_rows):
            r = self._conv(r, prefix + "/conv2", 3, stride, pad, act=ACT_RELU, bn_eps=BN_EPS, emit_h2=True, want_f32=False)
            if self._h2_input(r) is not None:
                return self._conv1x1_mean(r, prefix + "/conv3", mean_rows, act=ACT_RELU, bn_eps=BN_EPS, residual=shortcut)
            x = self._conv(r, prefix + "/conv3", 1, 1, act=ACT_RELU, bn_eps=BN_EPS, residual=shortcut, res_stride=1)
            out = self._sess.buf(self._tag + "/fc7", (x.shape[0], x.shape[-1]))
            return self._sess.mark("op:spatial_mean", 0, lambda: ops.spatial_mean(x, out=out), nbytes=4 * (x.numel() + out.numel()))
        c3_h2 = res_stride == 1 and self._h2_eligible(M3, depth, base, 1, prefix + "/conv3")
        r = self._conv(r, prefix + "/conv2", 3, stride, pad, act=ACT_RELU, bn_eps=BN_EPS, emit_h2=c3_h2, want_f32=not c3_h2)
        return self._conv(r, prefix + "/conv3", 1, 1, act=ACT_RELU, bn_eps=BN_EPS, residual=shortcut, res_stride=res_stride,
                          emit_h2=emit_out, want_f32=f32_out)

    def _trunk_planes_only(self, rows, base, next_stride, next_prefix=None):
        depth = 4 * base
        return (bool(cfg.HIP.H2_TRUNK_PLANES) and next_stride == 1
                and self._h2_eligible(rows, base, depth, 1, None if next_prefix is None else next_prefix + "/conv1")
                and self._h2_eligible(rows, depth, base, 1, None if next_prefix is None else next_prefix + "/conv3"))

    def _run_blocks(self, x, blocks, emit_last=True):
        for bi, (name, base, n_units, stride) in enumerate(blocks):
            for u in range(1, n_units + 1):
                s_u = stride if u == n_units else 1
                N, H, W, _ = x.shape
                rows = N * ops.conv_out_size(H, 3, s_u, 1, 1) * ops.conv_out_size(W, 3, s_u, 1, 1) if s_u > 1 else N * H * W
                planes_only = u < n_units and self._trunk_planes_only(rows, base, stride if u + 1 == n_units else 1,
                                                                       "%s/%s/unit_%d/bottleneck_v1" % (self._scope, name, u + 1))
                x = self._bottleneck(x, "%s/%s/unit_%d/bottleneck_v1" % (self._scope, name, u), base, s_u,
                                     emit_out=emit_last or u < n_units or bi + 1 < len(blocks), f32_out=not planes_only)
        return x

    def _crop_pool_layer(self, bottom, rois, name):
        return self._crop_pool(bottom, rois, name, max_pool=bool(cfg.RESNET.MAX_POOL))

    def _build_base(self):
        net = self._conv(self._image, self._scope + "/conv1", 7, 2, _same_pad(7, 2), act=ACT_RELU, bn_eps=BN_EPS,
                         fold_w=True, real_cin=3)
        N, H, W, C = net.shape
        out = self._sess.buf(self._tag + "/pool1", (N, ops.conv_out_size(H, 3, 2, 1, 1), ops.conv_out_size(W, 3, 2, 1, 1), C))
        self._sess.mark("op:maxpool", 0, lambda: ops.maxpool(net, 3, 2, (1, 1, 1, 1), out=out), nbytes=4 * (net.numel() + out.numel()))
        return self._wrote(out)

    def _image_to_head(self, is_training, reuse=None):
        assert (0 <= cfg.RESNET.FIXED_BLOCKS <= 3)
        net_conv = self._run_blocks(self._build_base(), self._blocks[0:3])
        self._act_summaries.append(net_conv)
        self._layers['head'] = net_conv
        return net_conv

    def _fused_tail_maps(self, net_conv):
        name = self._blocks[-1][0]
        prefix = "%s/%s/unit_1/bottleneck_v1" % (self._scope, name)
        sc_map = self._conv(net_conv, prefix + "/shortcut", 1, 1, act=ACT_NONE, bn_eps=BN_EPS, no_bias=True)
        c1_map = self._conv(net_conv, prefix + "/conv1", 1, 1, act=ACT_NONE, bn_eps=BN_EPS, no_bias=True)
        return sc_map, c1_map

    def _fused_tail_entry(self, net_conv, rois):
        sess, P = self._sess, cfg.POOLING_SIZE
        name, base, n_units, stride = self._blocks[-1]
        prefix = "%s/%s/unit_1/bottleneck_v1" % (self._scope, name)
        R = rois.shape[0]
        sc_map, c1_map = self._fused_tail_maps(net_conv)
        b_sc = sess.conv_info[prefix + "/shortcut"]["b"]
        b_c1 = sess.conv_info[prefix + "/conv1"]["b"]
        fs = float(self._feat_stride[0])
        sc_out = sess.buf(self._tag + "/" + prefix + "/shortcut_crop", (R, P, P, sc_map.shape[-1]))
        c1_out = sess.buf(self._tag + "/" + prefix + "/conv1_crop", (R, P, P, c1_map.shape[-1]))
        shortcut = self._crop_images(sc_map, rois, sc_out, bias=b_sc, act=ACT_NONE)
        r = self._crop_images(c1_map, rois, c1_out, bias=b_c1, act=ACT_RELU)
        c3_h2 = self._h2_eligible(R * P * P, 4 * base, base, 1, prefix + "/conv3")
        r = self._conv(r, prefix + "/conv2", 3, 1, (1, 1, 1, 1), act=ACT_RELU, bn_eps=BN_EPS, emit_h2=c3_h2, want_f32=not c3_h2)
        x = self._conv(r, prefix + "/conv3", 1, 1, act=ACT_RELU, bn_eps=BN_EPS, residual=shortcut, res_stride=1, emit_h2=n_units >= 2,
                       want_f32=not (n_units >= 2 and self._trunk_planes_only(R * P * P, base, stride if n_units == 2 else 1,
                                                                              "%s/%s/unit_2/bottleneck_v1" % (self._scope, name))))
        fused = stride == 1 and n_units >= 2 and self._mean_fusable(R * P * P, 4 * base, base, "%s/%s/unit_%d/bottleneck_v1/conv3" % (self._scope, name, n_units), P * P)
        for u in range(2, n_units + 1):
            x = self._bottleneck(x, "%s/%s/unit_%d/bottleneck_v1" % (self._scope, name, u), base, stride if u == n_units else 1,
                                 mean_rows=P * P if (fused and u == n_units) else 0, emit_out=u < n_units,
                                 f32_out=not (u < n_units and self._trunk_planes_only(R * P * P, base, stride if u + 1 == n_units else 1,
                                                                                      "%s/%s/unit_%d/bottleneck_v1" % (self._scope, name, u + 1))))
        if fused:
            return x
        out = sess.buf(self._tag + "/fc7", (x.shape[0], x.shape[-1]))
        return sess.mark("op:spatial_mean", 0, lambda: ops.spatial_mean(x, out=out), nbytes=4 * (x.numel() + out.numel()))

    def _head_to_tail(self, pool5, is_training, reuse=None):
        name, base, n_units, stride = self._blocks[-1]
        if stride == 1 and self._mean_fusable(pool5.shape[0] * pool5.shape[1] * pool5.shape[2], 4 * base, base,
                                              "%s/%s/unit_%d/bottleneck_v1/conv3" % (self._scope, name, n_units), pool5.shape[1] * pool5.shape[2]):
            x = pool5
            hw = pool5.shape[1] * pool5.shape[2]
            for u in range(1, n_units + 1):
                x = self._bottleneck(x, "%s/%s/unit_%d/bottleneck_v1" % (self._scope, name, u), base, 1, mean_rows=hw if u == n_units else 0)
            return x
        fc7 = self._run_blocks(pool5, self._blocks[-1:], emit_last=False)
# ... 13 lines not shown
```

Measured before the change: 554.6.

## Fuse bottleneck shortcut and conv3 1x1 GEMMs into one paired kernel

Adds paired GEMM kernels (h2 and x3 variants) that compute the projection shortcut and conv3 of a bottleneck unit's first block in one launch. Both K-loops accumulate into the same register tile, with the shortcut partial scaled and held in registers until the conv3 half finishes and the epilogue runs. This removes the f32 write and re-read of the shortcut tensor plus one kernel launch. It is enabled by default for block1 and block2 in test mode. The cost is more complex kernel scheduling and fixed tile choices for the pair path.

Measured after the change: 558.3 (median of 6 runs). No clear change (+0.7%).

```diff
diff --git a/include/frcnn_hip.h b/include/frcnn_hip.h
--- a/include/frcnn_hip.h
+++ b/include/frcnn_hip.h
@@ -193,12 +193,17 @@
 int frcnn_gemm_x3_pack(const float* w_d, int G, int N, int K, void* planes_d, void* stream);
 int frcnn_gemm_x3(const float* x_d, const void* planes_d, const float* bias_d, const float* res_d, float* y_d, int G, int M, int N,
                   int K, int act, int cfg, int terms, void* stream);
+int frcnn_gemm_x3_pair(const float* x1_d, const void* planes1_d, const float* bias1_d, int K1, const float* x2_d, const void* planes2_d,
+                       const float* bias2_d, int K2, float* y_d, int G, int M, int N, int act, int cfg, void* stream);
 size_t frcnn_h2_planes_bytes(long long rows, int K);
 int frcnn_h2_pack_w(const float* w_d, int G, int N, int K, void* planes_d, float* w_inv_d, void* stream);
 int frcnn_h2_split(const float* x_d, long long M, int K, void* planes_d, float* inv_d, void* stream);
 int frcnn_gemm_h2(const void* x_planes_d, const float* x_inv_d, const void* w_planes_d, const float* w_inv_d, const float* bias_d,
                   const float* res_d, const void* res_planes_d, const float* res_inv_d, float* y_d, void* y_planes_d, float* y_inv_d,
                   int G, int M, int N, int K, int act, int cfg, void* stream);
+int frcnn_gemm_h2_pair(const void* x1_planes_d, const float* x1_inv_d, const void* w1_planes_d, const float* w1_inv_d, const float* bias1_d,
+                       int K1, const void* x2_planes_d, const float* x2_inv_d, const void* w2_planes_d, const float* w2_inv_d,
+                       const float* bias2_d, int K2, float* y_d, void* y_planes_d, float* y_inv_d, int G, int M, int N, int act, void* stream);
 size_t frcnn_gemm_h2_mean_workspace_bytes(int G, int M, int N);
 int frcnn_gemm_h2_mean(const void* x_planes_d, const float* x_inv_d, const void* w_planes_d, const float* w_inv_d, const float* bias_d,
                        const float* res_d, const void* res_planes_d, const float* res_inv_d, int G, int M, int N, int K, int act, int rows,
diff --git a/scratch/shortcut_pair_time.py b/scratch/shortcut_pair_time.py
--- /dev/null
+++ b/scratch/shortcut_pair_time.py
@@ -0,0 +1,53 @@
+import os, sys, statistics
+ROOT = os.path.dirname(os.path.dirname(os.path.abspath(__file__)))
+sys.path.insert(0, os.path.join(ROOT, "tf-faster-rcnn_amd")); sys.path.insert(0, os.path.join(ROOT, "tf-faster-rcnn_amd", "lib"))
+import torch
+from frcnn_hip import ops
+dev = torch.device("cuda:0")
+g = torch.Generator(device=dev); g.manual_seed(1)
+ROUNDS, WARM = 50, 10
+def ev(): return torch.cuda.Event(enable_timing=True)
+def timed(fn):
+    a, z = ev(), ev(); a.record(); fn(); z.record(); return a, z
+def rnd(*s): return torch.randn(*s, device=dev, generator=g)
+def report(name, R, pairs):
+    for k in R: print("  %-22s median %7.1f us   min %7.1f us   (n = %d)" % (k, statistics.median(R[k]), min(R[k]), len(R[k])))
+    two = statistics.median(R["shortcut"]) + statistics.median(R["conv3"])
+    for k in pairs: print("  %s: two launches %.1f us (median sum), %s %.1f us = %.2f x, %+.1f us" % (name, two, k, statistics.median(R[k]), statistics.median(R[k]) / two, statistics.median(R[k]) - two))
+
+M, N, K1, K2 = 300000, 256, 64, 64
+x1, x2 = rnd(M, K1).clamp_(min=0), rnd(M, K2).clamp_(min=0)
+p1, p2 = ops.gemm_x3_pack(rnd(N, K1) / 8), ops.gemm_x3_pack(rnd(N, K2) / 8)
+b1, b2 = rnd(N), rnd(N)
+s, y0, y1 = (torch.empty(M, N, device=dev) for _ in range(3))
+R = {"shortcut": [], "conv3": [], "pair cfg 0 (64x128)": [], "pair cfg 1 (128x128)": []}
+for it in range(ROUNDS + WARM):
+    e = {}
+    e["shortcut"] = timed(lambda: ops.gemm_x3(x1, p1, 1, M, N, K1, b1, None, 0, out=s))
+    e["conv3"] = timed(lambda: ops.gemm_x3(x2, p2, 1, M, N, K2, b2, s, 1, out=y0))
+    e["pair cfg 0 (64x128)"] = timed(lambda: ops.gemm_x3_pair(x1, p1, b1, K1, x2, p2, b2, K2, 1, M, N, 1, out=y1, cfg=0))
+    e["pair cfg 1 (128x128)"] = timed(lambda: ops.gemm_x3_pair(x1, p1, b1, K1, x2, p2, b2, K2, 1, M, N, 1, out=y1, cfg=1))
+    torch.cuda.synchronize()
+    if it >= WARM:
+        for k, (a, z) in e.items(): R[k].append(a.elapsed_time(z) * 1000.0)
+print("block1 unit_1 (x3): M %d, %d -> %d and %d -> %d; bit equal: %s" % (M, K1, N, K2, N, torch.equal(y0, y1)))
+report("block1", R, ("pair cfg 0 (64x128)", "pair cfg 1 (128x128)"))
+del x1, x2, s, y0, y1
+
+for name, M, N, K1, K2 in (("block2", 75000, 512, 256, 128), ("block3", 19152, 1024, 512, 256)):
+    x1, x2 = ops.h2_split(rnd(M, K1).clamp_(min=0)), ops.h2_split(rnd(M, K2).clamp_(min=0))
+    w1, w2 = ops.h2_pack_w(rnd(N, K1) / 16), ops.h2_pack_w(rnd(N, K2) / 16)
+    b1, b2 = rnd(N), rnd(N)
+    s = torch.empty(M, N, device=dev)
+    yp0, yp1 = ops.H2.empty(M, N, dev), ops.H2.empty(M, N, dev)
+    R = {"shortcut": [], "conv3": [], "pair": []}
+    for it in range(ROUNDS + WARM):
+        e = {}
+        e["shortcut"] = timed(lambda: ops.gemm_h2(x1, w1, 1, M, N, K1, b1, None, 0, out=s))
+        e["conv3"] = timed(lambda: ops.gemm_h2(x2, w2, 1, M, N, K2, b2, s, 1, out_planes=yp0, want_f32=False))
+        e["pair"] = timed(lambda: ops.gemm_h2_pair(x1, w1, b1, x2, w2, b2, 1, M, N, 1, out_planes=yp1, want_f32=False))
+        torch.cuda.synchronize()
+        if it >= WARM:
+            for k, (a, z) in e.items(): R[k].append(a.elapsed_time(z) * 1000.0)
+    print("%s unit_1 (h2): M %d, %d -> %d and %d -> %d, planes out; bit equal: %s" % (name, M, K1, N, K2, N, torch.equal(yp0.planes, yp1.planes) and torch.equal(yp0.inv, yp1.inv)))
+    report(name, R, ("pair",))
diff --git a/tf-faster-rcnn_amd/csrc/gemm_h2.hip b/tf-faster-rcnn_amd/csrc/gemm_h2.hip
--- a/tf-faster-rcnn_amd/csrc/gemm_h2.hip
+++ b/tf-faster-rcnn_amd/csrc/gemm_h2.hip
@@ -15,6 +15,10 @@
   int wshare;
   const float* mask;
   float* mean_part; int mean_rows;
+};
+struct GemmH2PairParams : GemmH2Params {
+  const unsigned short* x2; const float* x2_inv; const unsigned short* w2; const float* w2_inv; const float* bias2;
+  int K2, nsteps2;
 };
 
 __device__ __forceinline__ void h2_glds16(unsigned voff, const void* sbase, unsigned lds_base) {
@@ -70,6 +74,7 @@
 enum H2Tune : int {
   H2_SCALES_ONCE = 2,
   H2_PINGPONG = 32,
+  H2_PAIR = 64,
   H2_MASKED = 128,
   H2_LIGHT_BOUNDARY = 256,
   H2_STORE16 = 512,
@@ -96,7 +101,8 @@
 };
 
 template <int BM, int BN, int WM, int WN, int NS, int WPE = 2, int TUNE = 0>
-__global__ __launch_bounds__((BM / WM) * (BN / WN) * 64) __attribute__((amdgpu_waves_per_eu(WPE))) void k_gemm_h2(const GemmH2Params p) {
+__global__ __launch_bounds__((BM / WM) * (BN / WN) * 64) __attribute__((amdgpu_waves_per_eu(WPE)))
+void k_gemm_h2(const std::conditional_t<(TUNE & H2_PAIR) != 0, GemmH2PairParams, GemmH2Params> p) {
   constexpr int NW = (BM / WM) * (BN / WN);
   constexpr int TM = WM / 32, TN = WN / 32;
   constexpr int LA = 2 * BM / 16 / NW;
@@ -109,6 +115,8 @@
   constexpr bool LTB = (TUNE & H2_LIGHT_BOUNDARY) != 0;
   constexpr bool W21 = (TUNE & H2_STORE16) != 0;
   constexpr bool DE = (TUNE & H2_DEFERRED) != 0;
+  constexpr bool PAIR = (TUNE & H2_PAIR) != 0;
+  static_assert(!PAIR || (LTB && !DE && !PP && !MASKED), "pair form: the standalone light boundary, where the residual sits raw in `tot` until the first fold");
   using L = H2Lds<BM, BN, WM, WN, NS, TUNE>;
   constexpr int XP = L::XP, WP = L::WP, S_OFF = L::S_OFF, STAGE = L::STAGE, RED_OFF = L::RED_OFF, S2_OFF = L::S2_OFF, CB_OFF = L::CB_OFF, RI_OFF = L::RI_OFF;
   static_assert(!LTB || (!PP && NS == 2 && NW >= 4 && BN % 64 == 0 && BM <= 128), "light boundary: the two-slot one-barrier-per-slab schedule");
@@ -129,7 +137,16 @@
   const int tile0 = t_end - tn + wx;
   if (tile0 >= t_end) return;
   const int my_tiles = (t_end - tile0 + W8 - 1) / W8;
+  auto op_x = [&](int h) { if constexpr (PAIR) { if (h) return p.x2; } return p.x; };
+  auto op_xinv = [&](int h) { if constexpr (PAIR) { if (h) return p.x2_inv; } return p.x_inv; };
+  auto op_w = [&](int h) { if constexpr (PAIR) { if (h) return p.w2; } return p.w; };
+  auto op_winv = [&](int h) { if constexpr (PAIR) { if (h) return p.w2_inv; } return p.w_inv; };
+  auto op_bias = [&](int h) { if constexpr (PAIR) { if (h) return p.bias2; } return p.bias; };
+  auto op_K = [&](int h) { if constexpr (PAIR) { if (h) return p.K2; } return p.K; };
+  auto op_nsteps = [&](int h) { if constexpr (PAIR) { if (h) return p.nsteps2; } return p.nsteps; };
+  int i_half = 0, c_half = 0;
   int left = __builtin_amdgcn_readfirstlane(my_tiles * p.nsteps);
+  if constexpr (PAIR) left = __builtin_amdgcn_readfirstlane(my_tiles * (p.nsteps + op_nsteps(1)));
 
   const int wmi = wave / (BN / WN), wni = wave % (BN / WN);
   const int wm0 = wmi * WM, wn0 = wni * WN;
@@ -158,6 +175,23 @@
     const int bm0 = mt * BM, bn0 = nt * BN;
     const size_t row0 = (size_t)g * p.M + bm0;
     i_g = g; i_bm0 = bm0; i_bn0 = bn0;
+    if constexpr (PAIR) {
+      const int K = op_K(i_half);
+      i_xb = (const char*)op_x(i_half) + row0 * K * 2;
+      i_wb = (const char*)op_w(i_half) + ((size_t)g * 2 * p.N + bn0) * K * 2;
+      i_sb = (const char*)(op_xinv(i_half) + row0);
+#pragma unroll
+      for (int t = 0; t < LA; ++t) {
+        const int u = wave * LA + t, plane = u / (BM / 16), row = (u % (BM / 16)) * 16 + (lane >> 2), pos = lane & 3;
+        const int rr = min(row, p.M - 1 - bm0);
+        a_off[t] = (unsigned)((size_t)plane * ((size_t)p.Mtot * K * 2) + (size_t)rr * K * 2 + ((pos ^ ((row >> 2) & 3)) * 16));
+      }
+#pragma unroll
+      for (int t = 0; t < LB; ++t) {
+        const int u = wave * LB + t, plane = u / (BN / 16), row = (u % (BN / 16)) * 16 + (lane >> 2), pos = lane & 3;
+        b_off[t] = (unsigned)((size_t)plane * ((size_t)p.N * K * 2) + (size_t)row * K * 2 + ((pos ^ ((row >> 2) & 3)) * 16));
+      }
+    } else {
     i_xb = (const char*)p.x + row0 * p.K * 2;
     i_wb = (const char*)p.w + ((size_t)(p.wshare ? 0 : g) * 2 * p.N + bn0) * p.K * 2;
     i_sb = (const char*)(p.x_inv + row0);
@@ -166,6 +200,7 @@
       const int u = wave * LA + t, plane = u / (BM / 16), row = (u % (BM / 16)) * 16 + (lane >> 2), pos = lane & 3;
       const int rr = min(row, p.M - 1 - bm0);
       a_off[t] = (unsigned)((size_t)plane * xplane + (size_t)rr * p.K * 2 + ((pos ^ ((row >> 2) & 3)) * 16));
+    }
     }
     const long long last = p.Mtot - 1 - (long long)row0;
 #pragma unroll
@@ -201,6 +236,19 @@
   };
   static_assert(!ONCE || NS == 2 || PP, "scales-once needs the uncounted wait of the two-stage ring");
   auto issue_advance = [&]() {
+    if constexpr (PAIR) {
+      --left;
+      if (++i_step == op_nsteps(i_half)) {
+        i_step = 0;
+        i_half ^= 1;
+        if (i_half == 0) i_tile += W8;
+        if (left > 0) set_tile(i_tile);
+      } else {
+        i_xb += 64; i_wb += 64;
+        if ((i_step & 3) == 0) i_sb += (size_t)p.Mtot * 4;
+      }
+      return;
+    }
     --left;
     if (++i_step == p.nsteps) {
       i_step = 0; i_tile += W8;
@@ -213,6 +261,21 @@
 
   auto issue_cb = [&]() {
     const unsigned cb = lds0 + CB_OFF + i_cpar * (2 * BN * 4);
+    if constexpr (PAIR) {
+      if (wave == 1) {
+#pragma unroll
+        for (int j = 0; j < BN / 64; ++j)
+          h2_glds4((unsigned)(lane * 4), uniform_ptr((const char*)(op_winv(i_half) + (size_t)i_g * p.N + i_bn0 + j * 64)),
+                   __builtin_amdgcn_readfirstlane(cb + j * 256));
+      }
+      if (wave == 2 && op_bias(i_half)) {
+#pragma unroll
+        for (int j = 0; j < BN / 64; ++j)
+          h2_glds4((unsigned)(lane * 4), uniform_ptr((const char*)(op_bias(i_half) + i_bn0 + j * 64)), __builtin_amdgcn_readfirstlane(cb + BN * 4 + j * 256));
+      }
+      i_cpar ^= 1;
+      return;
+    }
     if (wave == 1) {
 #pragma unroll
       for (int j = 0; j < BN / 64; ++j)
@@ -751,7 +814,7 @@
     if (fold) {
       if (LTB && first_block) {
         const float* cbp = (const float*)(smem + CB_OFF + c_cpar * (2 * BN * 4));
-        if (!p.res && p.resp) {
+        if (!PAIR && !p.res && p.resp) {
           typedef unsigned u32x2 __attribute__((ext_vector_type(2)));
 #pragma unroll
           for (int i = 0; i < TM; ++i) {
@@ -780,7 +843,7 @@
 #pragma unroll
           for (int q = 0; q < 4; ++q) {
             const float4 wi = *(const float4*)(cbp + wn0 + j * 32 + 4 * khalf + 8 * q);
-            const float4 bv = p.bias ? *(const float4*)(cbp + BN + wn0 + j * 32 + 4 * khalf + 8 * q) : make_float4(0.f, 0.f, 0.f, 0.f);
+            const float4 bv = (PAIR ? op_bias(c_half) : p.bias) ? *(const float4*)(cbp + BN + wn0 + j * 32 + 4 * khalf + 8 * q) : make_float4(0.f, 0.f, 0.f, 0.f);
             const float s0 = __uint_as_float(0x7f000000u - __float_as_uint(wi.x)), s1 = __uint_as_float(0x7f000000u - __float_as_uint(wi.y));
             const float s2 = __uint_as_float(0x7f000000u - __float_as_uint(wi.z)), s3 = __uint_as_float(0x7f000000u - __float_as_uint(wi.w));
 #pragma unroll
@@ -956,6 +1019,48 @@
       issue_advance();
       nxt = nxt + 1 == NS ? 0 : nxt + 1;
     }
+  }
+  if constexpr (PAIR) {
+    for (int vt = 0; vt < 2 * my_tiles; ++vt) {
+      if (c_half == 0) {
+#pragma unroll
+        for (int i = 0; i < TM; ++i)
+#pragma unroll
+          for (int j = 0; j < TN; ++j)
+#pragma unroll
+            for (int r = 0; r < 16; ++r) tot[i][j][r] = 0.f;
+      }
+      const int nk = op_nsteps(c_half) >> 2;
+      for (int kb = 0; kb < nk; ++kb) {
+        slab(std::integral_constant<int, 0>{}, false, kb == 0);
+        slab(std::integral_constant<int, 1>{}, false, kb == 0);
+        slab(std::integral_constant<int, 2>{}, false, kb == 0);
+        slab(std::integral_constant<int, 3>{}, true, kb == 0);
+      }
+      if (c_half == 0) {
+        const float* cbs = (const float*)(smem + CB_OFF + c_cpar * (2 * BN * 4));
+#pragma unroll
+        for (int j = 0; j < TN; ++j)
+#pragma unroll
+          for (int q = 0; q < 4; ++q) {
+            const float4 wi = *(const float4*)(cbs + wn0 + j * 32 + 4 * khalf + 8 * q);
+#pragma unroll
+            for (int i = 0; i < TM; ++i) {
+              tot[i][j][4 * q + 0] = tot[i][j][4 * q + 0] * wi.x; tot[i][j][4 * q + 1] = tot[i][j][4 * q + 1] * wi.y;
+              tot[i][j][4 * q + 2] = tot[i][j][4 * q + 2] * wi.z; tot[i][j][4 * q + 3] = tot[i][j][4 * q + 3] * wi.w;
+            }
+          }
+        c_cpar ^= 1;
+        c_half = 1;
+      } else {
+        epilogue(true);
+        c_half = 0;
+        c_tile += W8;
+        if (vt + 2 < 2 * my_tiles) set_ctile(c_tile);
+      }
+    }
+    h2_wait_vmcnt<0>();
+    return;
   }
   const int nkb = p.nsteps >> 2;
   for (int tl = 0; tl < my_tiles; ++tl) {
@@ -1228,3 +1333,36 @@
   LAUNCH_CHECK();
   return FRCNN_OK;
 }
+
+extern "C" int frcnn_gemm_h2_pair(const void* x1_planes_d, const float* x1_inv_d, const void* w1_planes_d, const float* w1_inv_d, const float* bias1_d,
+                                  int K1, const void* x2_planes_d, const float* x2_inv_d, const void* w2_planes_d, const float* w2_inv_d,
+                                  const float* bias2_d, int K2, float* y_d, void* y_planes_d, float* y_inv_d, int G, int M, int N, int act,
+                                  void* stream) {
+  if (!x1_planes_d || !x1_inv_d || !w1_planes_d || !w1_inv_d || !x2_planes_d || !x2_inv_d || !w2_planes_d || !w2_inv_d || (!y_d && !y_planes_d) ||
+      (y_planes_d && !y_inv_d) || G <= 0 || M <= 0 || N <= 0 || K1 <= 0 || K2 <= 0 || act < 0 || act > 2)
+    return FRCNN_E_ARG;
+  const long long Mtot = (long long)G * M;
+  const int Kmax = K1 > K2 ? K1 : K2;
+  if (K1 % H2_KB || K2 % H2_KB || N % 128 || 4ll * Mtot * Kmax >= (1ll << 32) || 4ll * N * Kmax >= (1ll << 32) || (long long)M * N >= (1ll << 29))
+    return FRCNN_E_UNSUPPORTED;
+  constexpr int TUNE = H2_SCALES_ONCE + H2_LIGHT_BOUNDARY + H2_STORE16 + H2_PAIR;
+  constexpr int BM = 128, BN = 128, NT = 256;
+  constexpr size_t lds = H2Lds<BM, BN, 64, 64, 2, TUNE>::TOTAL;
+  auto kern = k_gemm_h2<BM, BN, 64, 64, 2, 2, TUNE>;
+  static KernelOnce once;
+  int slots = 0;
+  HIP_TRY(kernel_once(once, (const void*)kern, NT, lds, &slots));
+  if (slots < 8) return FRCNN_E_UNSUPPORTED;
+  GemmH2PairParams p;
+  static_cast<GemmH2Params&>(p) = h2_params(x1_planes_d, x1_inv_d, w1_planes_d, w1_inv_d, bias1_d, nullptr, nullptr, nullptr, y_d, y_planes_d, y_inv_d,
+                                            G, M, N, K1, act);
+  p.x2 = (const unsigned short*)x2_planes_d; p.x2_inv = x2_inv_d; p.w2 = (const unsigned short*)w2_planes_d; p.w2_inv = w2_inv_d; p.bias2 = bias2_d;
+  p.K2 = K2;
+  p.mtiles = cdiv(M, BM); p.ntiles = N / BN; p.nsteps = K1 / 32; p.nsteps2 = K2 / 32;
+  const long long T = (long long)p.mtiles * p.ntiles * G;
+  if (T >= (1ll << 30)) return FRCNN_E_UNSUPPORTED;
+  const int grid = (int)min((long long)(slots / 8) * 8, ((T + 7) / 8) * 8);
+  hipLaunchKernelGGL(kern, dim3(grid), dim3(NT), lds, (hipStream_t)stream, p);
+  LAUNCH_CHECK();
+  return FRCNN_OK;
+}
diff --git a/tf-faster-rcnn_amd/csrc/gemm_x3.hip b/tf-faster-rcnn_amd/csrc/gemm_x3.hip
--- a/tf-faster-rcnn_amd/csrc/gemm_x3.hip
+++ b/tf-faster-rcnn_amd/csrc/gemm_x3.hip
@@ -1,6 +1,7 @@
 #include "common.h"
 #include "x3_mma.h"
 #include <mutex>
+#include <type_traits>
 
 struct GemmX3Params {
   const float* x; const unsigned short* wp; const float* bias; const float* res; float* y;
@@ -8,8 +9,14 @@
   long long gx, gwp, gy;
 };
 
-template <int BM, int BN, int WM, int WN, int TERMS = 6>
-__global__ __launch_bounds__((BM / WM) * (BN / WN) * 64) __attribute__((amdgpu_waves_per_eu(2))) void k_gemm_x3(const GemmX3Params p) {
+struct GemmX3PairParams : GemmX3Params {
+  const float* x2; const unsigned short* wp2; const float* bias2;
+  int K2, nsteps1;
+  long long gx2, gwp2;
+};
+
+template <int BM, int BN, int WM, int WN, int TERMS = 6, bool PAIR = false>
+__global__ __launch_bounds__((BM / WM) * (BN / WN) * 64) __attribute__((amdgpu_waves_per_eu(2))) void k_gemm_x3(const std::conditional_t<PAIR, GemmX3PairParams, GemmX3Params> p) {
   constexpr int NW = (BM / WM) * (BN / WN);
   constexpr int TM = WM / 32, TN = WN / 32;
   constexpr int LA = BM / 8 / NW;
@@ -49,6 +56,14 @@
       const int row = (wave * LA + t) * 8 + (lane >> 3);
       a_lane[t] = (min(row, p.M - 1 - i_bm0) * p.K + ((lane & 7) ^ ((row >> 1) & 7)) * 4) * 4;
     }
+    if constexpr (PAIR) {
+#pragma unroll
+      for (int t = 0; t < LB; ++t) {
+        const int u = wave * LB + t;
+        const int plane = u / (BN / 16), row = (u % (BN / 16)) * 16 + (lane >> 2), pos = lane & 3;
+        b_lane[t] = ((plane * p.N + row) * p.K) * 2 + ((pos ^ ((row >> 2) & 3)) * 16);
+      }
+    }
   };
   const unsigned lds0 = (unsigned)(size_t)(LDS_AS char*)smem;
   auto issue_one = [&](int buf, int t) {
@@ -56,6 +71,23 @@
     if (t < LA) glds16((const char*)ia + a_lane[t], __builtin_amdgcn_readfirstlane(sb + (wave * LA + t) * 1024));
     else glds16(ib + b_lane[t - LA], __builtin_amdgcn_readfirstlane(sb + A_BYTES + (wave * LB + (t - LA)) * 1024));
   };
+  auto set_phase2 = [&]() {
+    if constexpr (PAIR) {
+      ia = p.x2 + (size_t)i_g * p.gx2 + (size_t)i_bm0 * p.K2;
+      ib = (const char*)(p.wp2 + (size_t)i_g * p.gwp2 + (size_t)i_bn0 * p.K2);
+#pragma unroll
+      for (int t = 0; t < LA; ++t) {
+        const int row = (wave * LA + t) * 8 + (lane >> 3);
+        a_lane[t] = (min(row, p.M - 1 - i_bm0) * p.K2 + ((lane & 7) ^ ((row >> 1) & 7)) * 4) * 4;
+      }
+#pragma unroll
+      for (int t = 0; t < LB; ++t) {
+        const int u = wave * LB + t;
+        const int plane = u / (BN / 16), row = (u % (BN / 16)) * 16 + (lane >> 2), pos = lane & 3;
+        b_lane[t] = ((plane * p.N + row) * p.K2) * 2 + ((pos ^ ((row >> 2) & 3)) * 16);
+      }
+    }
+  };
   auto advance_k = [&]() { ia += 32; ib += 64; };
   auto issue_slab = [&](int buf) {
 #pragma unroll
@@ -73,6 +105,8 @@
         for (int r = 0; r < 16; ++r) { acc[i][j][r] = 0.f; acs[i][j][r] = 0.f; }
   };
   zero_acc();
+  f32x16 sreg[PAIR ? TM : 1][PAIR ? TN : 1];
+  (void)sreg;
   const int frow = lane & 31, khalf = lane >> 5;
   const int a_sw = (frow >> 1) & 7, b_sw = (frow >> 2) & 3;
   const int a_row = (wm0 + frow) * 128, b_row = A_BYTES + (wn0 + frow) * 64;
@@ -128,7 +162,9 @@
     for (int i = 0; i < TM; ++i)
 #pragma unroll
       for (int j = 0; j < TN; ++j) {
-        const float bv = p.bias ? p.bias[c_bn0 + wn0 + j * 32 + frow] : 0.f;
+        float bv;
+        if constexpr (PAIR) bv = p.bias2 ? p.bias2[c_bn0 + wn0 + j * 32 + frow] : 0.f;
+        else bv = p.bias ? p.bias[c_bn0 + wn0 + j * 32 + frow] : 0.f;
         const long long sbase = sub_base(i, j);
         float v[16];
         if (RES) {
@@ -140,12 +176,26 @@
         for (int r = 0; r < 16; ++r) {
           float t = (acc[i][j][r] + acs[i][j][r]) + bv;
           if (RES) t += v[r];
+          if constexpr (PAIR) t += sreg[i][j][r];
           v[r] = act_clamp(t, act_lo, act_hi);
         }
         const auto ry = rsrc_of(py, sbase);
 #pragma unroll
         for (int r = 0; r < 16; ++r) __builtin_amdgcn_raw_buffer_store_b32(__builtin_bit_cast(unsigned, v[r]), ry, lo + row_soff(r), 0, 0);
       }
+  };
+
+  auto hold_s = [&]() {
+    if constexpr (PAIR) {
+#pragma unroll
+      for (int i = 0; i < TM; ++i)
+#pragma unroll
+        for (int j = 0; j < TN; ++j) {
+          const float bv = p.bias ? p.bias[c_bn0 + wn0 + j * 32 + frow] : 0.f;
+#pragma unroll
+          for (int r = 0; r < 16; ++r) sreg[i][j][r] = (acc[i][j][r] + acs[i][j][r]) + bv;
+        }
+    }
   };
 
   set_tile(tile);
@@ -161,10 +211,13 @@
       next = __builtin_amdgcn_readfirstlane(tile + W8);
       set_tile(next < t_end ? next : tile);
     }
+    if constexpr (PAIR) { if (step + 1 == p.nsteps1) set_phase2(); }
     slab_body(cur);
     cur ^= 1;
+    if constexpr (PAIR) { if (step + 1 == p.nsteps1) { hold_s(); zero_acc(); } }
     if (!last) { ++step; continue; }
-    if (p.res) finish(std::true_type{}); else finish(std::false_type{});
+    if constexpr (PAIR) finish(std::false_type{});
+    else if (p.res) finish(std::true_type{}); else finish(std::false_type{});
     if (next >= t_end) break;
     zero_acc();
     step = 0; tile = next; c_bm0 = i_bm0; c_bn0 = i_bn0; c_g = i_g;
@@ -250,3 +303,42 @@
     default: return FRCNN_E_ARG;
   }
 }
+
+template <int BM, int BN, int WM, int WN>
+static int launch_x3_pair(const GemmX3PairParams& q, hipStream_t st) {
+  constexpr int NT = (BM / WM) * (BN / WN) * 64;
+  constexpr size_t lds = 2 * (size_t)(BM * 128 + 3 * BN * 64);
+  auto kern = k_gemm_x3<BM, BN, WM, WN, 6, true>;
+  static KernelOnce once;
+  int slots = 0;
+  HIP_TRY(kernel_once(once, (const void*)kern, NT, lds, &slots));
+  if (slots < 8 || q.N % BN) return FRCNN_E_UNSUPPORTED;
+  GemmX3PairParams p = q;
+  p.mtiles = cdiv(p.M, BM); p.ntiles = p.N / BN; p.nsteps1 = p.K / 32; p.nsteps = p.nsteps1 + p.K2 / 32;
+  const long long T = (long long)p.mtiles * p.ntiles * p.batch;
+  if (T >= (1ll << 30)) return FRCNN_E_UNSUPPORTED;
+  const int grid = (int)min((long long)(slots / 8) * 8, ((T + 7) / 8) * 8);
+  hipLaunchKernelGGL(kern, dim3(grid), dim3(NT), lds, st, p);
+  LAUNCH_CHECK();
+  return FRCNN_OK;
+}
+
+extern "C" int frcnn_gemm_x3_pair(const float* x1_d, const void* planes1_d, const float* bias1_d, int K1, const float* x2_d,
+                                  const void* planes2_d, const float* bias2_d, int K2, float* y_d, int G, int M, int N, int act, int cfg,
+                                  void* stream) {
+  if (!x1_d || !planes1_d || !x2_d || !planes2_d || !y_d || G <= 0 || M <= 0 || N <= 0 || K1 <= 0 || K2 <= 0 || act < 0 || act > 2 || cfg < -1 || cfg > 1)
+    return FRCNN_E_ARG;
+  const int Kmax = K1 > K2 ? K1 : K2;
+  if (K1 % 32 || K2 % 32 || N % 128 || (long long)M * N >= (1ll << 31) || (long long)N * Kmax >= (1ll << 28) || Kmax >= (1 << 22))
+    return FRCNN_E_UNSUPPORTED;
+  GemmX3PairParams p;
+  p.x = x1_d; p.wp = (const unsigned short*)planes1_d; p.bias = bias1_d; p.res = nullptr; p.y = y_d;
+  p.M = M; p.N = N; p.K = K1; p.batch = G; p.act = act;
+  p.gx = (long long)M * K1; p.gwp = 3ll * N * K1; p.gy = (long long)M * N;
+  p.x2 = x2_d; p.wp2 = (const unsigned short*)planes2_d; p.bias2 = bias2_d; p.K2 = K2;
+  p.gx2 = (long long)M * K2; p.gwp2 = 3ll * N * K2;
+  p.nsteps = p.nsteps1 = p.mtiles = p.ntiles = 0;
+  hipStream_t st = (hipStream_t)stream;
+  if (cfg < 0) cfg = 1;
+  return cfg == 0 ? launch_x3_pair<64, 128, 32, 64>(p, st) : launch_x3_pair<128, 128, 32, 64>(p, st);
+}
diff --git a/tf-faster-rcnn_amd/frcnn_hip/__init__.py b/tf-faster-rcnn_amd/frcnn_hip/__init__.py
--- a/tf-faster-rcnn_amd/frcnn_hip/__init__.py
+++ b/tf-faster-rcnn_amd/frcnn_hip/__init__.py
@@ -152,11 +152,13 @@
     "frcnn_gemm_x3_pack_bytes": (c_size_t, [c_int, c_int, c_int]),
     "frcnn_gemm_x3_pack": (c_int, [_P, c_int, c_int, c_int, _P, _P]),
     "frcnn_gemm_x3": (c_int, [_P, _P, _P, _P, _P, c_int, c_int, c_int, c_int, c_int, c_int, c_int, _P]),
+    "frcnn_gemm_x3_pair": (c_int, [_P, _P, _P, c_int, _P, _P, _P, c_int, _P, c_int, c_int, c_int, c_int, c_int, _P]),
     "frcnn_h2_planes_bytes": (c_size_t, [c_longlong, c_int]),
     "frcnn_h2_pack_w": (c_int, [_P, c_int, c_int, c_int, _P, _P, _P]),
     "frcnn_h2_split": (c_int, [_P, c_longlong, c_int, _P, _P, _P]),
     "frcnn_gemm_h2": (c_int, [_P, _P, _P, _P, _P, _P, _P, _P, _P, _P, _P, c_int, c_int, c_int, c_int, c_int, c_int, _P]),
-    "frcnn_gemm_h2_mean_workspace_bytes": (c_size_t, [c_int, c_int, c_int]),
+    "frcnn_gemm_h2_pair": (c_int, [_P, _P, _P, _P, _P, c_int, _P, _P, _P, _P, _P, c_int, _P, _P, _P, c_int, c_int, c_int, c_int, _P]),
+    "frcnn_gemm_h2_mean_workspace_bytes":(c_size_t, [c_int, c_int, c_int]),
     "frcnn_gemm_h2_mean": (c_int, [_P, _P, _P, _P, _P, _P, _P, _P, c_int, c_int, c_int, c_int, c_int, c_int, _P, _P, c_size_t, c_int, _P]),
     "frcnn_relu6_bwd": (c_int, [_P, _P, c_longlong, _P]),
     "frcnn_maxpool_bwd": (c_int, [_P, c_int, c_int, c_int, c_int, c_int, c_int, _P, _P, c_int, c_int, _P, _P]),
diff --git a/tf-faster-rcnn_amd/frcnn_hip/ops.py b/tf-faster-rcnn_amd/frcnn_hip/ops.py
--- a/tf-faster-rcnn_amd/frcnn_hip/ops.py
+++ b/tf-faster-rcnn_amd/frcnn_hip/ops.py
@@ -1163,6 +1163,14 @@
     return out
 
 
+def gemm_x3_pair(x1, planes1, bias1, K1, x2, planes2, bias2, K2, G, M, N, act=ACT_NONE, out=None, cfg=-1):
+    _chk(x1), _chk(x2)
+    out = _empty((G, M, N) if G > 1 else (M, N), dtype=torch.float32, device=x1.device) if out is None else out
+    call("frcnn_gemm_x3_pair", _ptr(x1), _ptr(planes1), _ptr(bias1), int(K1), _ptr(x2), _ptr(planes2), _ptr(bias2), int(K2), _ptr(out),
+         int(G), int(M), int(N), int(act), int(cfg), _stream())
+    return out
+
+
 class H2(object):
     __slots__ = ("planes", "inv", "rows", "K")
 
@@ -1224,6 +1232,19 @@
     return out, out_planes
 
 
+def gemm_h2_pair(x1, wp1, bias1, x2, wp2, bias2, G, M, N, act=ACT_NONE, out=None, out_planes=None, want_f32=True):
+    assert isinstance(x1, H2) and isinstance(x2, H2) and x1.rows == G * M and x2.rows == G * M
+    if out is None and want_f32:
+        out = _empty((G * M, N), dtype=torch.float32, device=x1.planes.device)
+    if out_planes is not None:
+        assert out_planes.rows == G * M and out_planes.K == N
+    call("frcnn_gemm_h2_pair", _ptr(x1.planes), _ptr(x1.inv), _ptr(wp1[0]), _ptr(wp1[1]), _ptr(bias1), int(x1.K),
+         _ptr(x2.planes), _ptr(x2.inv), _ptr(wp2[0]), _ptr(wp2[1]), _ptr(bias2), int(x2.K), _ptr(out),
+         _ptr(None if out_planes is None else out_planes.planes), _ptr(None if out_planes is None else out_planes.inv),
+         int(G), int(M), int(N), int(act), _stream())
+    return out, out_planes
+
+
 def gemm_h2_mean(x, wp, G, M, N, K, bias, residual, act, rows, out=None, cfg=-1):
     assert isinstance(x, H2) and x.rows == G * M and x.K == K and M % rows == 0
     if out is None:
diff --git a/tf-faster-rcnn_amd/lib/model/config.py b/tf-faster-rcnn_amd/lib/model/config.py
--- a/tf-faster-rcnn_amd/lib/model/config.py
+++ b/tf-faster-rcnn_amd/lib/model/config.py
@@ -55,7 +55,7 @@
              WINOGRAD_TRAIN=True, WINOGRAD_DGRAD=True,
              WINOGRAD_7X7=True, WINOGRAD_FUSED_F2=True, FUSE_TAIL_MEAN=True, MFMA_X3=True,
              MFMA_H2=True, H2_LAZY_SPLIT=True, H2_MIN_TILES=150, H2_TRAIN_MIN_TILES=320, H2_TRUNK_PLANES=True, H2_TILE_CFG=-1,
-             X3_TILE_CFG=-1, H2_TRAIN=True, WGRAD_STREAM=2, WGRAD_TN=True, WGRAD_H2=True, PREP_STREAM=True, TRAIN_REPLAY=True, TRAIN_PICK_STREAMS=6,
+             X3_TILE_CFG=-1, FUSE_SHORTCUT=("block1", "block2"), X3_PAIR_CFG=-1, H2_TRAIN=True, WGRAD_STREAM=2, WGRAD_TN=True, WGRAD_H2=True, PREP_STREAM=True, TRAIN_REPLAY=True, TRAIN_PICK_STREAMS=6,
              GRAPH_CACHE_SHAPES=4, TRAIN_CACHE_SHAPES=16, JPEG_DEVICE=False, TEST_BATCH_IMAGES=1,
              SOFT_NMS=0, SOFT_NMS_SIGMA=0.5, SOFT_NMS_MIN_SCORE=0.001, TEST_FLIP=False, BBOX_VOTE=False, BBOX_VOTE_THRESH=0.8))
 __C.DATA_DIR = osp.abspath(osp.join(__C.ROOT_DIR, 'data'))
diff --git a/tf-faster-rcnn_amd/lib/nets/network.py b/tf-faster-rcnn_amd/lib/nets/network.py
--- a/tf-faster-rcnn_amd/lib/nets/network.py
+++ b/tf-faster-rcnn_amd/lib/nets/network.py
@@ -132,6 +132,34 @@
                 self._requires_grad.add(out.data_ptr())
         return out
 
+    def _conv1x1_pair(self, x, r, sc_scope, c3_scope, pipe, act=ACT_RELU, bn_eps=None, emit_h2=False, want_f32=True):
+        sess = self._sess
+        w1, b1 = sess.conv_params(sc_scope, bn_eps=bn_eps)
+        w2, b2 = sess.conv_params(c3_scope, bn_eps=bn_eps)
+        N, H, W, K1 = x.shape
+        K2, Cout = r.shape[-1], w2.shape[0]
+        M = N * H * W
+        assert tuple(r.shape[:3]) == (N, H, W) and w1.shape[0] == Cout
+        out = sess.buf(self._tag + "/" + c3_scope, (N, H, W, Cout))
+        flops = 2 * M * Cout * (K1 + K2)
+        if pipe == "h2":
+            xp1, xp2 = self._h2_input(x), self._h2_input(r)
+            wp1, wp2 = sess.h2_planes(w1), sess.h2_planes(w2)
+            yp = sess.h2_buf(self._tag + "/" + c3_scope, M, Cout) if emit_h2 else None
+            y = out if (want_f32 or yp is None) else None
+            sess.mark("conv:h2:pair:" + c3_scope, flops,
+                      lambda: ops.gemm_h2_pair(xp1, wp1, b1, xp2, wp2, b2, 1, M, Cout, act, out=y, out_planes=yp, want_f32=False),
+                      nbytes=4 * M * (K1 + K2) + 4 * (w1.numel() + w2.numel()) + (4 * out.numel() if y is not None else 0)
+                      + (4 * out.numel() if yp is not None else 0))
+            return self._wrote(out, yp, y is not None)
+        self._need_f32(x), self._need_f32(r)
+        p1, p2 = sess.x3_planes(w1), sess.x3_planes(w2)
+        xc = int(cfg.HIP.X3_PAIR_CFG)
+        sess.mark("conv:x3:pair:" + c3_scope, flops,
+                  lambda: ops.gemm_x3_pair(x, p1, b1, K1, r, p2, b2, K2, 1, M, Cout, act, out=out, cfg=xc),
+                  nbytes=4 * (x.numel() + r.numel() + out.numel()) + 6 * (w1.numel() + w2.numel()))
+        return self._wrote(out)
+
     H2_MIN_CHANNEL_RATIO = 2.0 ** -18
 
     def _h2_eligible(self, M, N, K, G, scope=None):
@@ -606,7 +634,8 @@
                 c.RPN_PRE_NMS_TOP_N, c.RPN_POST_NMS_TOP_N, c.RPN_NMS_THRESH, cfg.TEST.RPN_TOP_N, cfg.POOLING_SIZE,
                 bool(cfg.HIP.WINOGRAD), int(cfg.HIP.WINOGRAD_MIN_CIN), int(cfg.HIP.WINOGRAD_M), tuple(cfg.HIP.WINOGRAD_F2_SCOPES),
                 tuple(cfg.HIP.WINOGRAD_DIRECT_SCOPES), bool(cfg.HIP.WINOGRAD_7X7), bool(cfg.HIP.FUSE_TAIL_MEAN), bool(cfg.HIP.MFMA_X3), bool(cfg.USE_E2E_TF),
-                bool(cfg.HIP.MFMA_H2), bool(cfg.HIP.H2_LAZY_SPLIT), int(cfg.HIP.H2_MIN_TILES), bool(cfg.HIP.H2_TRUNK_PLANES), int(cfg.HIP.H2_TILE_CFG), int(cfg.HIP.X3_TILE_CFG), bool(cfg.HIP.H2_TRAIN))
+                bool(cfg.HIP.MFMA_H2), bool(cfg.HIP.H2_LAZY_SPLIT), int(cfg.HIP.H2_MIN_TILES), bool(cfg.HIP.H2_TRUNK_PLANES), int(cfg.HIP.H2_TILE_CFG), int(cfg.HIP.X3_TILE_CFG), bool(cfg.HIP.H2_TRAIN),
+                tuple(cfg.HIP.FUSE_SHORTCUT), int(cfg.HIP.X3_PAIR_CFG))
 
     def shape_scope(self, sess, image_shape, im_info):
         return sess.shape_scope(self.graph_key(image_shape, im_info), group=("graphs", self._tag), cap=int(cfg.HIP.GRAPH_CACHE_SHAPES))
diff --git a/tf-faster-rcnn_amd/lib/nets/resnet_v1.py b/tf-faster-rcnn_amd/lib/nets/resnet_v1.py
--- a/tf-faster-rcnn_amd/lib/nets/resnet_v1.py
+++ b/tf-faster-rcnn_amd/lib/nets/resnet_v1.py
@@ -54,8 +54,10 @@
     def _bottleneck(self, x, prefix, base, stride, mean_rows=0, emit_out=True, f32_out=True):
         depth = base * 4
         cin = x.shape[-1]
+        pair = None
         if cin != depth:
-            shortcut = self._conv(x, prefix + "/shortcut", 1, stride, act=ACT_NONE, bn_eps=BN_EPS)
+            pair = None if mean_rows else self._shortcut_pair_pipe(x, prefix, base, stride)
+            shortcut = None if pair else self._conv(x, prefix + "/shortcut", 1, stride, act=ACT_NONE, bn_eps=BN_EPS)
             res_stride = 1
         else:
             shortcut, res_stride = x, stride
@@ -72,8 +74,26 @@
             return self._sess.mark("op:spatial_mean", 0, lambda: ops.spatial_mean(x, out=out), nbytes=4 * (x.numel() + out.numel()))
         c3_h2 = res_stride == 1 and self._h2_eligible(M3, depth, base, 1, prefix + "/conv3")
         r = self._conv(r, prefix + "/conv2", 3, stride, pad, act=ACT_RELU, bn_eps=BN_EPS, emit_h2=c3_h2, want_f32=not c3_h2)
+        if pair == "h2" and self._h2_input(r) is None:
+            pair, shortcut = None, self._conv(x, prefix + "/shortcut", 1, stride, act=ACT_NONE, bn_eps=BN_EPS)
+        if pair:
+            return self._conv1x1_pair(x, r, prefix + "/shortcut", prefix + "/conv3", pair, act=ACT_RELU, bn_eps=BN_EPS,
+                                      emit_h2=emit_out, want_f32=f32_out)
         return self._conv(r, prefix + "/conv3", 1, 1, act=ACT_RELU, bn_eps=BN_EPS, residual=shortcut, res_stride=res_stride,
                           emit_h2=emit_out, want_f32=f32_out)
+
+    def _shortcut_pair_pipe(self, x, prefix, base, stride):
+        block = prefix[len(self._scope) + 1:].split("/")[0]
+        if self._mode != "TEST" or stride != 1 or block not in tuple(cfg.HIP.FUSE_SHORTCUT):
+            return None
+        N, H, W, cin = x.shape
+        M, depth = N * H * W, 4 * base
+        sc_h2 = self._h2_eligible(M, depth, cin, 1, prefix + "/shortcut") and self._h2_input(x) is not None
+        sc = "h2" if sc_h2 else "x3" if self._x3_eligible(M, depth, cin, 1) else None
+        c3 = "h2" if self._h2_eligible(M, depth, base, 1, prefix + "/conv3") else "x3" if self._x3_eligible(M, depth, base, 1) else None
+        if sc is None or sc != c3 or (sc == "x3" and (depth % 128 or x.data_ptr() in self._f32_missing)):
+            return None
+        return sc
 
     def _trunk_planes_only(self, rows, base, next_stride, next_prefix=None):
         depth = 4 * base
```
